# liuQuan98/EYOC

Hardware: AMD Instinct MI355X
Metric: registered pairs/sec (30k-voxel KITTI pairs) (higher is better)
Workload: dtype f32 (split16 products: fp32 storage/accumulation, 3 fp16 MFMAs on hi/lo-split operands per product); 1 GPU; 64 synthetic 30 cm KITTI-shaped pairs per step per GPU (mean 29894 voxels/cloud, ResUNetBN2C random-init, 5000-point NN, RANSAC 4000000 hypotheses/pair, planted inlier ratio 0.3, spconv math split16); parallelism=pairs sharded over 1 GPU(s), steps_in_flight=2

## Files before the change

### eyoc_amd/_lib.py

```python
from __future__ import annotations

import ctypes as C
import os
import threading

_HERE = os.path.dirname(os.path.abspath(__file__))
LIB_PATH = os.environ.get("EYOC_HIP_LIB") or os.path.join(_HERE, "lib", "libeyoc_hip.so")

MAX_LEVELS = 4
MAP_S1, MAP_DOWN, MAP_UP = 0, 1, 2


class MapsInfo(C.Structure):
    _fields_ = [("n_levels", C.c_int32), ("rows", C.c_int32 * MAX_LEVELS),
                ("pairs_s1", C.c_int64 * MAX_LEVELS), ("pairs_down", C.c_int64 * MAX_LEVELS),
                ("pairs_up", C.c_int64 * MAX_LEVELS), ("pairs_conv1", C.c_int64)]


class ModelDesc(C.Structure):
    _fields_ = [("in_channels", C.c_int32), ("out_channels", C.c_int32), ("conv1_kernel_size", C.c_int32),
                ("normalize_feature", C.c_int32), ("channels", C.c_int32 * 5), ("tr_channels", C.c_int32 * 5),
                ("bn_eps", C.c_float), ("expanded", C.c_int32)]


class LayerParams(C.Structure):
    _fields_ = [("name", C.c_char_p), ("kernel", C.POINTER(C.c_float)), ("K", C.c_int32), ("cin", C.c_int32),
                ("cout", C.c_int32), ("bias", C.POINTER(C.c_float)), ("bn_weight", C.POINTER(C.c_float)),
                ("bn_bias", C.POINTER(C.c_float)), ("bn_mean", C.POINTER(C.c_float)),
                ("bn_var", C.POINTER(C.c_float))]


class RansacParams(C.Structure):
    _fields_ = [("max_distance", C.c_float), ("edge_similarity", C.c_float), ("max_iteration", C.c_int32),
                ("seed", C.c_uint32)]


class RansacResult(C.Structure):
    _fields_ = [("T", C.c_float * 16), ("inliers", C.c_int32), ("best_hypothesis", C.c_int32),
                ("survivors", C.c_int32), ("inlier_rmse", C.c_float)]


class Sc2pcrParams(C.Structure):
    _fields_ = [("inlier_threshold", C.c_float), ("d_thre", C.c_float), ("ratio", C.c_float),
                ("nms_radius", C.c_float), ("num_iterations", C.c_int32), ("max_points", C.c_int32),
                ("k1", C.c_int32), ("k2", C.c_int32)]


_vp, _i, _sz = C.c_void_p, C.c_int, C.c_size_t
PROTOTYPES = {
    "eyoc_version": (_i, []),
    "eyoc_last_error": (C.c_char_p, []),
    "eyoc_create": (_i, [_i, C.POINTER(_vp)]),
    "eyoc_destroy": (_i, [_vp]),
    "eyoc_maps_workspace_bytes": (_sz, [_i]),
    "eyoc_maps_build": (_i, [_vp, _vp, _i, _vp, _sz, _vp, C.POINTER(_vp)]),
    "eyoc_maps_build_ordered": (_i, [_vp, _vp, _i, _vp, _sz, _vp, _i, C.POINTER(_vp)]),
    "eyoc_maps_free": (_i, [_vp]),
    "eyoc_maps_last_fault_batches": (_i, [_vp, _vp, _vp]),
    "eyoc_maps_internal_order": (_i, [_vp, _i]),
    "eyoc_maps_lazy_tables": (_i, [_vp, _i]),
    "eyoc_maps_fused_levels": (_i, [_vp, _i]),
    "eyoc_spconv_select_down_kernel": (_i, [_vp, _i]),
    "eyoc_maps_order_window_shift": (_i, [_vp, _i]),
    "eyoc_maps_row_order": (_vp, [_vp]),
    "eyoc_maps_copy_row_order": (_i, [_vp, _vp, _vp]),
    "eyoc_maps_rows": (_i, [_vp, _i]),
    "eyoc_maps_coords": (_vp, [_vp, _i]),
    "eyoc_maps_table": (_vp, [_vp, _i, _i]),
    "eyoc_maps_copy_coords": (_i, [_vp, _i, _vp, _vp]),
    "eyoc_maps_copy_table": (_i, [_vp, _i, _i, _vp, _vp]),
    "eyoc_maps_copy_up_order": (_i, [_vp, _i, _vp, _vp]),
    "eyoc_maps_order_min_rows": (_i, [_vp, _i]),
    "eyoc_maps_info": (_i, [_vp, _vp, _i, _vp, C.POINTER(MapsInfo)]),
    "eyoc_voxelize_workspace_bytes": (_sz, [_i]),
    "eyoc_voxelize": (_i, [_vp, _vp, _i, _i, C.c_float, _i, _vp, _vp, C.POINTER(C.c_int), _vp, _sz, _vp]),
    "eyoc_voxelize_batched_workspace_bytes": (_sz, [_i, _i]),
    "eyoc_voxelize_batched": (_i, [_vp, _vp, _i, C.POINTER(C.c_int64), _i, _i, C.c_float, _i, _vp, _vp, _vp,
                                   C.POINTER(C.c_int64), _vp, _sz, _vp]),
    "eyoc_voxelize_batched_isolating_workspace_bytes": (_sz, [_i, _i]),
    "eyoc_voxelize_batched_isolating": (_i, [_vp, _vp, _i, C.POINTER(C.c_int64), _i, _i, C.c_float, _i, _vp, _vp, _vp,
                                             C.POINTER(C.c_int64), _vp, _sz, _vp, _vp]),
    "eyoc_batch_drop_workspace_bytes": (_sz, [_i]),
    "eyoc_batch_drop": (_i, [_vp, _vp, _vp, _i, _i, _vp, _vp, _vp, _vp, C.POINTER(C.c_int), _vp, _vp, _sz, _vp]),
    "eyoc_remap_rows": (_i, [_vp, _vp, _i, _vp, _i, _vp, _vp]),
    "eyoc_gather_rows": (_i, [_vp, _vp, _i, _i, _vp, _i, _vp, C.c_float, _vp, _vp]),
    "eyoc_dotmax": (_i, [_vp, _vp, _vp, _i, C.POINTER(C.c_int32), C.POINTER(C.c_int32), _i, _vp, _vp, _vp]),
    "eyoc_knn2": (_i, [_vp, _vp, _vp, _i, C.POINTER(C.c_int32), C.POINTER(C.c_int32), _i, _vp, _vp, _vp, _vp]),
    "eyoc_lowe_topk": (_i, [_vp, _vp, _vp, _i, _i, _vp, _vp, _vp]),
    "eyoc_pair_filter": (_i, [_vp, _i, _vp, _vp, _vp, _vp, _i, _vp, C.c_float, _vp, _vp, _vp]),
    "eyoc_pair_filter_similarity": (_i, [_vp, _vp, _vp, _vp, _vp, _i, _vp, _i, _i, C.c_float, C.c_float, C.c_double, _vp, _vp,
                                         _vp]),
    "eyoc_spconv_packed_floats": (_sz, [_i, _i, _i]),
    "eyoc_spconv_pack_weights": (_i, [_vp, _vp, _i, _i, _i, _vp]),
    "eyoc_spconv_select_kernel": (_i, [_vp, _i]),
    "eyoc_spconv_pack_weights_transposed": (_i, [_vp, _i, _i, _i, _i, _vp]),
    "eyoc_spconv_grad_weight_workspace_bytes": (_sz, [_i, _i, _i, _i]),
    "eyoc_spconv_grad_weight": (_i, [_vp, _vp, _i, _i, _vp, _i, _i, _vp, _i, _i, _vp, _vp, _sz, _vp]),
    "eyoc_spconv_pack_weights_split16": (_i, [_vp, _vp, _i, _i, _i, _vp, _vp]),
    "eyoc_spconv_ex": (_i, [_vp, _vp, _i, _i, _i, _vp, _i, _i, _vp, _i, _vp, _vp, _i, _i, _vp, _i, _i, _i, _vp, _vp]),
    "eyoc_spconv_select_split16_kernel": (_i, [_vp, _i]),
    "eyoc_spconv_select_st_kernel": (_i, [_vp, _i]),
    "eyoc_spconv_st_split_below": (_i, [_vp, _i]),
    "eyoc_spconv_st_group_rows": (_i, [_vp, _i]),
    "eyoc_spconv_st_ksplit": (_i, [_vp, _i]),
    "eyoc_spconv_local_rulebook_bytes": (_sz, [_i]),
    "eyoc_spconv_build_local_rulebook": (_i, [_vp, _vp, _i, _i, _vp, _vp, _vp]),
    "eyoc_spconv_staged": (_i, [_vp, _vp, _vp, _i, _i, _vp, _i, _i, _vp, _i, _vp, _vp, _i, _i, _vp, _i, _i, _vp, _vp]),
    "eyoc_split16_encode": (_i, [_vp, _vp, _i, _i, _i, _vp, _i, _vp]),
    "eyoc_split16_decode": (_i, [_vp, _vp, _i, _i, _i, _vp, _i, _vp]),
    "eyoc_model_set_math": (_i, [_vp, _i]),
    "eyoc_model_last_math": (_i, [_vp]),
    "eyoc_model_range_check": (_i, [_vp, _vp, C.POINTER(C.c_float)]),
    "eyoc_model_range_snapshot": (_i, [_vp, _vp, _vp]),
    "eyoc_model_set_progress_event": (_i, [_vp, _i, _vp]),
    "eyoc_model_set_probe": (_i, [_vp, _i]),
    "eyoc_spconv": (_i, [_vp, _vp, _i, _i, _vp, _i, _i, _vp, _i, _vp, _vp, _i, _i, _vp, _i, _vp]),
    "eyoc_spconv_sum": (_i, [_vp, _vp, _i, _i, _vp, _i, _i, _vp, _i, _vp, _i, _vp]),
    "eyoc_model_blob_floats": (_sz, [C.POINTER(ModelDesc)]),
    "eyoc_model_pack_host": (_i, [C.POINTER(ModelDesc), C.POINTER(LayerParams), _i, _vp, _sz]),
    "eyoc_model_create": (_i, [_vp, C.POINTER(ModelDesc), C.POINTER(LayerParams), _i, _vp, _sz, C.POINTER(_vp)]),
    "eyoc_model_destroy": (_i, [_vp]),
    "eyoc_model_fuse_tail": (_i, [_vp, _i]),
    "eyoc_model_workspace_bytes": (_sz, [_vp, _vp]),
    "eyoc_model_forward": (_i, [_vp, _vp, _vp, _vp, _vp, _vp, _sz, _vp]),
    "eyoc_model_num_layers": (_i, [_vp]),
    "eyoc_model_layer_work": (_i, [_vp, _vp, _vp, _vp, C.POINTER(C.c_char_p), C.POINTER(C.c_int64),
                                   C.POINTER(C.c_double), C.POINTER(C.c_double), C.POINTER(C.c_double)]),
    "eyoc_model_set_timing": (_i, [_vp, _i]),
    "eyoc_model_layer_ms": (_i, [_vp, C.POINTER(C.c_float)]),
    "eyoc_model_timing_slot": (_i, [_vp, _i]),
    "eyoc_bn_workspace_bytes": (_sz, [_i, _i]),
    "eyoc_bn_train_forward": (_i, [_vp, _vp, _i, _i, _i, _vp, _vp, C.c_float, _i, _vp, _i, _vp, _vp, _sz, _vp]),
    "eyoc_bn_train_forward_running": (_i, [_vp, _vp, _i, _i, _i, _vp, _vp, C.c_float, _i, _vp, _i, _vp, _vp, _vp, C.c_float, _vp, _sz, _vp]),
    "eyoc_bn_train_backward": (_i, [_vp, _vp, _i, _vp, _i, _vp, _i, _i, _i, _vp, _vp, C.c_float, _vp, _i, _vp, _vp, _vp, _sz, _vp]),
    "eyoc_maps_gather_window": (_i, [_vp, _vp, _i, _vp, _i, _vp, _vp]),
    "eyoc_maps_gather_window_internal": (_i, [_vp, _vp, _i, _vp, _i, _vp, _vp]),
    "eyoc_knn_prefilter": (_i, [_vp, _i]),
    "eyoc_spconv_select_up_kernel": (_i, [_vp, _i]),
    "eyoc_spconv_upc_min_rows": (_i, [_vp, _i]),
    "eyoc_spconv_upc_tile_rows": (_i, [_i, _i]),
    "eyoc_spconv_upc_bytes": (_sz, [_i]),
    "eyoc_spconv_upc_build": (_i, [_vp, _vp, _i, _vp, _vp, _vp]),
    "eyoc_spconv_upc": (_i, [_vp, _vp, _vp, _i, _i, _vp, _i, _i, _vp, _i, _vp, _i, _vp, _i, _i, _vp, _vp]),
    "eyoc_spconv_select_conv1_kernel": (_i, [_vp, _i]),
    "eyoc_knn1": (_i, [_vp, _vp, _vp, _i, C.POINTER(C.c_int32), C.POINTER(C.c_int32), _i, _i, _vp, _vp, _vp]),
    "eyoc_pdist": (_i, [_vp, _vp, _i, _vp, _i, _i, _i, _vp, _vp]),
    "eyoc_kabsch_batched": (_i, [_vp, _vp, _vp, _vp, _i, _i, _vp, _vp]),
    "eyoc_irls_quad": (_i, [_vp, _vp, _vp, _vp, _i, _i, _vp, _vp]),
    "eyoc_ransac": (_i, [_vp, _vp, _vp, _vp, _i, C.POINTER(RansacParams), _vp, _vp]),
    "eyoc_maps_select_orders": (_i, [_vp, _i, _i]),
    "eyoc_ransac_select_pruning": (_i, [_vp, _i]),
    "eyoc_registration_accept_degenerate": (_i, [_vp, _i]),
    "eyoc_ransac_transform_store": (_i, [_vp, _i]),
    "eyoc_ransac_workspace_bytes": (_sz, [_vp, _i, _i, _i, _sz]),
    "eyoc_ransac_batched_ws": (_i, [_vp, _vp, _vp, _vp, C.POINTER(C.c_int32), C.POINTER(C.c_int32), _i,
                                    C.POINTER(RansacParams), _vp, _vp, _sz, _vp]),
    "eyoc_ransac_batched": (_i, [_vp, _vp, _vp, _vp, C.POINTER(C.c_int32), C.POINTER(C.c_int32), _i,
                                 C.POINTER(RansacParams), _vp, _vp]),
    "eyoc_sc2pcr_workspace_bytes": (_sz, [_i, C.POINTER(Sc2pcrParams)]),
    "eyoc_sc2pcr": (_i, [_vp, _vp, _vp, _i, C.POINTER(Sc2pcrParams), _vp, _vp, _vp, _sz, _vp]),
    "eyoc_sc2pcr_batched_workspace_bytes": (_sz, [_i, C.POINTER(Sc2pcrParams)]),
    "eyoc_sc2pcr_batched_workspace_bytes_n": (_sz, [_i, _i, C.POINTER(Sc2pcrParams)]),
    "eyoc_sc2pcr_set_shortlist_cap": (_i, [_vp, _i]),
    "eyoc_sc2pcr_set_dense_threshold": (_i, [_vp, _i]),
    "eyoc_sc2pcr_select_kernels": (_i, [_vp, _i]),
    "eyoc_sc2pcr_batched": (_i, [_vp, _vp, _vp, C.POINTER(C.c_int32), _i, C.POINTER(Sc2pcrParams), _vp, _vp, _i, _vp, _sz,
                                 _vp]),
}


ERR_INVALID, ERR_HIP, ERR_WORKSPACE, ERR_DUPLICATE, ERR_RANGE = -1, -2, -3, -4, -5


class EyocError(RuntimeError):

    def __init__(self, msg, code=None):
        super().__init__(msg)
        self.code = code


_lib = None
_lock = threading.Lock()
_ctx = {}


def load():
    global _lib
    if _lib is not None:
        return _lib
    with _lock:
        if _lib is None:
            if not os.path.exists(LIB_PATH):
                raise EyocError(
                    f"{LIB_PATH} not found: build it with `python -m eyoc_amd.build` (hipcc, gfx950). "
                    "There is no CPU fallback for this path.")
            lib = C.CDLL(LIB_PATH)
            for name, (res, args) in PROTOTYPES.items():
                fn = getattr(lib, name)
                fn.restype, fn.argtypes = res, args
            _lib = lib
    return _lib


def check(rc: int, what: str = ""):
    if rc != 0:
        msg = load().eyoc_last_error().decode("utf-8", "replace")
        raise EyocError(f"{what or 'libeyoc_hip'} failed ({rc}): {msg}", rc)


def ctx(device_index: int | None = None):
    import torch
    if device_index is not None:
        h = _ctx.get(device_index)
        if h is not None:
# ... 93 lines not shown
```

### eyoc_amd/csrc/common.h

```cpp
#pragma once
#include <hip/hip_runtime.h>

#include <cstdarg>
#include <cstdint>
#include <cstdio>
#include <cstring>
#include <string>
#include <vector>

#include "../../include/eyoc_hip.h"

namespace eyoc {

void set_error(const char* fmt, ...);

#define EYOC_CHECK_HIP(expr)                                                               \
  do {                                                                                     \
    hipError_t _e = (expr);                                                                \
    if (_e != hipSuccess) {                                                                \
      eyoc::set_error("%s failed: %s (%s:%d)", #expr, hipGetErrorString(_e), __FILE__,    \
                      __LINE__);                                                           \
      return EYOC_ERR_HIP;                                                                 \
    }                                                                                      \
  } while (0)

#define EYOC_REQUIRE(cond, code, ...)  \
  do {                                 \
    if (!(cond)) {                     \
      eyoc::set_error(__VA_ARGS__);    \
      return (code);                   \
    }                                  \
  } while (0)

inline size_t align_up(size_t v, size_t a = 256) { return (v + a - 1) / a * a; }
inline int cdiv(long long a, long long b) { return (int)((a + b - 1) / b); }

struct Carver {
  char* base;
  size_t off = 0, cap;
  Carver(void* p, size_t bytes) : base((char*)p), cap(bytes) {}
  template <typename T>
  T* take(size_t count) {
    size_t o = align_up(off);
    off = o + count * sizeof(T);
    return (T*)(base ? base + o : nullptr);
  }
  bool ok() const { return off <= cap; }
};

}

struct eyoc_ctx {
  int device = 0;
  void* scratch = nullptr;
  size_t scratch_bytes = 0;
  void* pinned = nullptr;
  size_t pinned_bytes = 0;
  int ensure_scratch(size_t bytes, hipStream_t st);
  hipStream_t scratch_owner = nullptr;
  bool scratch_owned = false;
  hipEvent_t scratch_ev = nullptr;
  static constexpr int POOL = 8;
  hipStream_t pool[POOL] = {};
  hipEvent_t pool_done[POOL] = {};
  hipEvent_t pool_fork = nullptr;
  bool pool_ready = false;
  int ensure_pool();
  bool ransac_attr_set = false, sc2_attr_set = false;
  bool up_attr_set[2] = {false, false};
  int zorder_kbits = 17, zorder_bbits = 10;
  int sc2_list_cap = 1024, sc2_dense_x = 0;
  int sc2_legacy = 0;
  uint32_t fault_dup[32] = {}, fault_range[32] = {};
  struct Knobs {
    int maps_order_min_rows = 65536;
    int maps_window_shift = 18;
    int maps_s1_order = 1, maps_down_order = 0;
    int maps_internal_order = -1;
    int maps_lazy_tables = 1, maps_fused_levels = 1;
    int knn_prefilter = 1;
    int fuse_tail = 2;
    int spconv_kernel = -1;
    int split16_kernel = 1;
    int up_kernel = 2;
    int s1_wide = 1;
    int st128_wide = 1;
    int down_kernel = 1;
    int upc_min_rows = 1 << 17;
    int conv1_kernel = 1;
    int st_group = 1;
    int st_variant = 1;
    int st_split_below = 1024;
    int st_cg_local = 1;
    int st_ksplit = 1;
    int ransac_store = 1 << 20;
    int ransac_prune = 2;
    int accept_degenerate = 0;
  } knobs;
};
inline const eyoc_ctx::Knobs& knobs_of(const eyoc_ctx* ctx) {
  static const eyoc_ctx::Knobs defaults;
  return ctx ? ctx->knobs : defaults;
}

namespace eyoc {

constexpr unsigned long long KEY_EMPTY = 0xFFFFFFFFFFFFFFFFull;
constexpr int COORD_BIAS = 1 << 17;
constexpr int VAL_UNSET = 0x7F7F7F7F;

struct HashTable {
  unsigned long long* keys;
  int* vals;
  unsigned int mask;
};

__host__ __device__ inline unsigned long long pack_key(int b, int x, int y, int z) {
  return ((unsigned long long)(unsigned)b << 54) |
         ((unsigned long long)((unsigned)(x + COORD_BIAS) & 0x3FFFFu) << 36) |
         ((unsigned long long)((unsigned)(y + COORD_BIAS) & 0x3FFFFu) << 18) |
         ((unsigned long long)((unsigned)(z + COORD_BIAS) & 0x3FFFFu));
}

__host__ __device__ inline unsigned int hash_key(unsigned long long k) {
  k ^= k >> 33;
  k *= 0xff51afd7ed558ccdull;
  k ^= k >> 33;
  k *= 0xc4ceb9fe1a85ec53ull;
  k ^= k >> 33;
  return (unsigned int)k;
}

__device__ inline int hash_lookup(const HashTable& t, unsigned long long key) {
  unsigned int s = hash_key(key) & t.mask;
  for (unsigned int probes = 0; probes <= t.mask; ++probes) {
    unsigned long long k = t.keys[s];
    if (k == key) return t.vals[s];
    if (k == KEY_EMPTY) return -1;
    s = (s + 1) & t.mask;
  }
  return -1;
}

}

struct eyoc_maps {
  int n_levels = 0;
  int rows[EYOC_MAX_LEVELS] = {0, 0, 0, 0};
  int32_t* coords[EYOC_MAX_LEVELS] = {nullptr, nullptr, nullptr, nullptr};
  eyoc::HashTable table[EYOC_MAX_LEVELS];
  int32_t* nbr_s1[EYOC_MAX_LEVELS] = {nullptr, nullptr, nullptr, nullptr};
  int32_t* nbr_down[EYOC_MAX_LEVELS] = {nullptr, nullptr, nullptr, nullptr};
  int32_t* nbr_up[EYOC_MAX_LEVELS] = {nullptr, nullptr, nullptr, nullptr};
  int32_t* parent[EYOC_MAX_LEVELS] = {nullptr, nullptr, nullptr, nullptr};
  int32_t* children[EYOC_MAX_LEVELS] = {nullptr, nullptr, nullptr, nullptr};
  int32_t* perm_up[EYOC_MAX_LEVELS] = {nullptr, nullptr, nullptr, nullptr};
  int32_t* perm_s1[EYOC_MAX_LEVELS] = {nullptr, nullptr, nullptr, nullptr};
  int32_t* perm_down[EYOC_MAX_LEVELS] = {nullptr, nullptr, nullptr, nullptr};
  int32_t* row_perm = nullptr;
  unsigned char* local_s1[EYOC_MAX_LEVELS] = {nullptr, nullptr, nullptr, nullptr};
  unsigned char* local_up[EYOC_MAX_LEVELS] = {nullptr, nullptr, nullptr, nullptr};
  unsigned char* local_s1w[EYOC_MAX_LEVELS] = {nullptr, nullptr, nullptr, nullptr};
  unsigned char* local_down[EYOC_MAX_LEVELS] = {nullptr, nullptr, nullptr, nullptr};
  unsigned char* local_upc[EYOC_MAX_LEVELS] = {nullptr, nullptr, nullptr, nullptr};
  bool table0_built = false;
  bool s1_ready[EYOC_MAX_LEVELS] = {true, true, true, true};
  bool up_ready[EYOC_MAX_LEVELS] = {true, true, true, true};
  int32_t* up8[EYOC_MAX_LEVELS] = {nullptr, nullptr, nullptr, nullptr};
  hipEvent_t s1_ev[EYOC_MAX_LEVELS] = {nullptr, nullptr, nullptr, nullptr};
  hipEvent_t up_ev[EYOC_MAX_LEVELS] = {nullptr, nullptr, nullptr, nullptr};
  hipEvent_t table0_ev = nullptr;
  eyoc_maps() = default;
  eyoc_maps(const eyoc_maps&) = delete;
  eyoc_maps& operator=(const eyoc_maps&) = delete;
  ~eyoc_maps();
};

namespace eyoc {
int maps_build_table0(eyoc_maps* maps, hipStream_t st);
int maps_ensure_table(eyoc_maps* maps, int kind, int level, hipStream_t st);
size_t sort_rows64_tmp_bytes(int n);
int sort_rows_by_key64(void* tmp, size_t tmp_bytes, const unsigned long long* keys_in, unsigned long long* keys_out, const int* vals_in,
                       int* vals_out, int n, int bits, hipStream_t st);
size_t sort_rows_tmp_bytes(int n, int bits);
int sort_rows_by_key(void* tmp, size_t tmp_bytes, const unsigned int* keys_in, unsigned int* keys_out, const int* vals_in,
                     int* vals_out, int n, int bits, hipStream_t st);
}
```

### eyoc_amd/csrc/coordmap.hip

```cpp
#include <cstdlib>

#include "spconv.h"
#include "derive.h"
#include "scan.h"

using namespace eyoc;

namespace {

__device__ inline void coarse_coord(const int32_t* c, int ts2, int& b, int& x, int& y, int& z) {
  const int m = ~(ts2 - 1);
  b = c[0]; x = c[1] & m; y = c[2] & m; z = c[3] & m;
}

__global__ void k_insert(const int32_t* __restrict__ coords, int n, int ts2, HashTable t, int* __restrict__ slot_out,
                         int* __restrict__ err, unsigned int* __restrict__ range_mask = nullptr) {
  int i = blockIdx.x * blockDim.x + threadIdx.x;
  if (i >= n) return;
  int b, x, y, z;
  coarse_coord(coords + 4 * (size_t)i, ts2, b, x, y, z);
  constexpr int LIM = COORD_BIAS - 16;
  if (b < 0 || b >= 1024 || x < -LIM || x >= LIM || y < -LIM || y >= LIM || z < -LIM || z >= LIM) {
    if (err) atomicAdd(&err[0], 1);
    if (range_mask && b >= 0 && b < 1024) atomicOr(&range_mask[b >> 5], 1u << (b & 31));
// ... 764 lines not shown
      hipLaunchKernelGGL(k_flag_sorted, dim3(cdiv(n_src, 256)), dim3(256), 0, st, src, n_src, ts2, flag,
                         l == 1 ? counters : (int*)nullptr, l == 1 ? counters + 1 : (int*)nullptr);
    } else {
      const unsigned int cap = table_capacity(n_src);
      t.keys = cv.take<unsigned long long>(cap);
      t.vals = cv.take<int>(cap);
      t.mask = cap - 1;
      FAIL_HIP(hipMemsetAsync(t.keys, 0xFF, (size_t)cap * 8, st));
      FAIL_HIP(hipMemsetAsync(t.vals, 0x7F, (size_t)cap * 4, st));
      hipLaunchKernelGGL(k_insert, dim3(cdiv(n_src, 256)), dim3(256), 0, st, src, n_src, ts2, t, slot, counters,
                         l == 1 ? fault_masks + 32 : (unsigned int*)nullptr);
      hipLaunchKernelGGL(k_flag, dim3(cdiv(n_src, 256)), dim3(256), 0, st, slot, t.vals, n_src, flag, (int*)nullptr);
    }
    hipLaunchKernelGGL(k_scan_partials, dim3(nb), dim3(SCAN_BLOCK), 0, st, flag, n_src, partial);
    hipLaunchKernelGGL(k_scan_top, dim3(1), dim3(SCAN_BLOCK), 0, st, partial, nb, counters + 2 + l);
    if (zorder) {
      m->rows[l] = pre_rows[l];
    } else {
    if (l == 1) {
      FAIL_HIP(hipMemcpyAsync(host + 128, counters, 128 * sizeof(int), hipMemcpyDeviceToHost, st));
      FAIL_HIP(hipStreamSynchronize(st));
      host[0] = host[128 + 2 + l]; host[1] = host[128]; host[2] = host[128 + 1];
    } else {
      FAIL_HIP(hipMemcpyAsync(host, counters + 2 + l, sizeof(int), hipMemcpyDeviceToHost, st));
      FAIL_HIP(hipStreamSynchronize(st));
    }
    if (l == 1 && host[1] != 0) {
      set_error("eyoc_maps_build: %d coordinate rows outside the supported key range (|c| < 2^17 - 16, 0 <= batch < 1024)", host[1]);
      keep_fault_masks(ctx, host + 128 + 64, EYOC_ERR_RANGE);
      delete m;
      return EYOC_ERR_RANGE;
    }
    if (l == 1 && sorted_level && host[2] != 0) {
      set_error("eyoc_maps_build: %d duplicate coordinate rows (a sparse tensor needs unique coordinates)", host[2]);
      keep_fault_masks(ctx, host + 128 + 64, EYOC_ERR_DUPLICATE);
      delete m;
      return EYOC_ERR_DUPLICATE;
    }
    m->rows[l] = host[0];
    }
    m->coords[l] = cv.take<int32_t>((size_t)m->rows[l] * 4);
    m->parent[l - 1] = cv.take<int32_t>((size_t)n_src);
    if (!zorder) {
      m->children[l - 1] = cv.take<int32_t>((size_t)m->rows[l] * 8);
      FAIL_HIP(hipMemsetAsync(m->children[l - 1], 0xFF, (size_t)m->rows[l] * 32, st));
    }
    if (sorted_level) {
      hipLaunchKernelGGL(k_compact_sorted, dim3(nb), dim3(SCAN_BLOCK), 0, st, flag, partial, src, n_src, ts2, l - 1,
                         m->coords[l], m->parent[l - 1], m->children[l - 1]);
      if (l + 1 == EYOC_MAX_LEVELS) {
        hipLaunchKernelGGL(k_insert, dim3(cdiv(m->rows[l], 256)), dim3(256), 0, st, m->coords[l], m->rows[l], ts2, t, (int*)nullptr, counters);
      }
      continue;
    }
    hipLaunchKernelGGL(k_compact<false>, dim3(nb), dim3(SCAN_BLOCK), 0, st, flag, partial, slot, src, n_src, ts2,
                       m->coords[l], t.vals, (int32_t*)nullptr);
    hipLaunchKernelGGL(k_children, dim3(cdiv(n_src, 256)), dim3(256), 0, st, slot, t.vals, src, n_src, l - 1,
                       m->parent[l - 1], m->children[l - 1], l == 1 ? counters + 1 : (int*)nullptr,
                       l == 1 ? fault_masks : (unsigned int*)nullptr);
    if (l == 1) {
      FAIL_HIP(hipMemcpyAsync(host + 128, counters, 128 * sizeof(int), hipMemcpyDeviceToHost, st));
      FAIL_HIP(hipStreamSynchronize(st));
      host[0] = host[128 + 1];
      if (host[0] != 0) {
        set_error("eyoc_maps_build: %d duplicate coordinate rows (a sparse tensor needs unique coordinates)", host[0]);
        keep_fault_masks(ctx, host + 128 + 64, EYOC_ERR_DUPLICATE);
        delete m;
        return EYOC_ERR_DUPLICATE;
      }
    }
  }
  const bool use_upc = kn.up_kernel == 2 && n >= kn.upc_min_rows;
  const bool use_up = kn.up_kernel == 1 || (kn.up_kernel == 2 && !use_upc);
  const bool lazy = zorder && use_upc && kn.maps_lazy_tables != 0;
  for (int l = 0; l < EYOC_MAX_LEVELS; ++l) {
    m->nbr_s1[l] = cv.take<int32_t>((size_t)27 * m->rows[l]);
    if (l + 1 < EYOC_MAX_LEVELS) {
      m->nbr_down[l] = cv.take<int32_t>((size_t)27 * m->rows[l + 1]);
      m->nbr_up[l] = cv.take<int32_t>((size_t)27 * m->rows[l]);
      if (lazy) {
        m->up8[l] = cv.take<int32_t>((size_t)8 * m->rows[l]);
        m->up_ready[l] = false;
      }
    }
  }
  if (lazy) m->s1_ready[0] = false;
  {
    const int top = EYOC_MAX_LEVELS - 1;
    hipLaunchKernelGGL(k_neighbours, dim3(cdiv(m->rows[top], 256)), dim3(256), 0, st, m->coords[top], m->rows[top],
                       m->table[top], 1 << top, 1, m->nbr_s1[top]);
  }
  const bool s1_order = kn.maps_s1_order != 0;
  int seg_up[EYOC_MAX_LEVELS], seg_s1[EYOC_MAX_LEVELS], seg_dn[EYOC_MAX_LEVELS], seg_base[3 * EYOC_MAX_LEVELS], n_seg = 0;
  size_t total = 0;
  for (int l = 0; l < EYOC_MAX_LEVELS; ++l) {
    seg_up[l] = seg_s1[l] = seg_dn[l] = -1;
    const bool dn_order = kn.maps_down_order == 1;
    if (l + 1 < EYOC_MAX_LEVELS && m->rows[l + 1] >= kn.maps_order_min_rows && (dn_order || !zorder)) {
      seg_dn[l] = n_seg; seg_base[n_seg++] = (int)total; total += m->rows[l + 1];
    }
    if (m->rows[l] < kn.maps_order_min_rows) continue;
    if (l + 1 < EYOC_MAX_LEVELS && !(zorder && (use_up || use_upc))) { seg_up[l] = n_seg; seg_base[n_seg++] = (int)total; total += m->rows[l]; }
    if (s1_order && !zorder) { seg_s1[l] = n_seg; seg_base[n_seg++] = (int)total; total += m->rows[l]; }
  }
  constexpr int TAG_SHIFT = UP_KEY_BITS, TAG_BITS = 4;
  const int wshift = zorder ? kn.maps_window_shift : -1;
  unsigned int* key_in = cv.take<unsigned int>(total);
  unsigned int* key_out = cv.take<unsigned int>(total);
  int* row_in = cv.take<int>(total);
  int32_t* perm_all = cv.take<int32_t>(total);
  const size_t sort_bytes = sort_rows_tmp_bytes((int)total, TAG_SHIFT + TAG_BITS);
  void* sort_tmp = cv.take<char>(sort_bytes);
  for (int l = EYOC_MAX_LEVELS - 2; l >= 0; --l) {
    const int nl = m->rows[l], nc = m->rows[l + 1];
    const int su = seg_up[l];
    if (lazy) {
      if (l > 0)
        hipLaunchKernelGGL((k_derive_fine<true, 2>), dim3(cdiv(nl, 256)), dim3(256), 0, st, m->coords[l], nl, l, m->parent[l], m->children[l],
                           m->nbr_s1[l + 1], nc, m->nbr_s1[l], m->up8[l], (unsigned int*)nullptr, (int*)nullptr, 0u, wshift);
    } else {
      hipLaunchKernelGGL((k_derive_fine<true, 1>), dim3(cdiv(nl, 256)), dim3(256), 0, st, m->coords[l], nl, l, m->parent[l],
                         m->children[l], m->nbr_s1[l + 1], nc, m->nbr_s1[l], m->nbr_up[l],
                         su >= 0 ? key_in + seg_base[su] : (unsigned int*)nullptr, su >= 0 ? row_in + seg_base[su] : (int*)nullptr,
                         (unsigned int)(su >= 0 ? su : 0) << TAG_SHIFT, wshift);
    }
    hipLaunchKernelGGL(k_derive_down, dim3(cdiv(nc, 256)), dim3(256), 0, st, nc, m->children[l], m->nbr_s1[l + 1],
                       m->nbr_down[l]);
  }
  for (int l = 0; l + 1 < EYOC_MAX_LEVELS; ++l) {
    const int sd = seg_dn[l];
    if (sd < 0) continue;
    hipLaunchKernelGGL(k_children_key, dim3(cdiv(m->rows[l + 1], 256)), dim3(256), 0, st, m->children[l], m->rows[l + 1],
                       key_in + seg_base[sd], row_in + seg_base[sd], (unsigned int)sd << TAG_SHIFT, wshift);
  }
  for (int l = 0; l < EYOC_MAX_LEVELS; ++l) {
    const int ss = seg_s1[l];
    if (ss < 0) continue;
    const int bits = l == 0 ? 2 : 4;
    hipLaunchKernelGGL(k_pattern_key, dim3(cdiv(m->rows[l], 256)), dim3(256), 0, st, m->nbr_s1[l], m->rows[l], bits,
                       key_in + seg_base[ss], row_in + seg_base[ss], (unsigned int)ss << TAG_SHIFT, wshift);
  }
  if (total > 0) {
    if (int rc = sort_rows_by_key(sort_tmp, sort_bytes, key_in, key_out, row_in, perm_all, (int)total, TAG_SHIFT + TAG_BITS, st)) {
      delete m;
      return rc;
    }
    for (int l = 0; l < EYOC_MAX_LEVELS; ++l) {
      if (seg_up[l] >= 0) m->perm_up[l] = perm_all + seg_base[seg_up[l]];
      if (seg_s1[l] >= 0) m->perm_s1[l] = perm_all + seg_base[seg_s1[l]];
      if (seg_dn[l] >= 0) m->perm_down[l] = perm_all + seg_base[seg_dn[l]];
    }
  }
  if (zorder) {
    for (int l = 0; l < EYOC_MAX_LEVELS; ++l) {
      m->local_s1[l] = cv.take<unsigned char>(local_rulebook_bytes(m->rows[l]));
      if (lazy && l == 0) {
        DeriveSrc src;
        src.coords = m->coords[0]; src.parent = m->parent[0]; src.children = m->children[0]; src.s1c = m->nbr_s1[1];
        src.nc = m->rows[1]; src.sh = 0; src.up8 = m->up8[0];
        if (int rc = build_local_rulebook_derived(src, m->rows[0], m->local_s1[0], counters + 8, st, kn.st_group)) { delete m; return rc; }
      } else if (int rc = build_local_rulebook(m->nbr_s1[l], 27, m->rows[l], m->local_s1[l], counters + 8, st, kn.st_group)) { delete m; return rc; }
      if (l + 1 < EYOC_MAX_LEVELS && use_up) {
        m->local_up[l] = cv.take<unsigned char>(local_rulebook_up_bytes(m->rows[l]));
        if (int rc = build_local_rulebook_up(m->nbr_up[l], 27, m->rows[l], m->local_up[l], counters + 9, st)) { delete m; return rc; }
      }
      if (l + 1 < EYOC_MAX_LEVELS && use_upc) {
        m->local_upc[l] = cv.take<unsigned char>(upc_kept_bytes(m->rows[l]));
        unsigned char* scratch = cv.take<unsigned char>(upc_scratch_bytes(m->rows[l]));
        if (m->local_upc[l]) {
          if (int rc = build_upc(lazy ? m->up8[l] : m->nbr_up[l], m->coords[l], 1 << l, m->rows[l], m->local_upc[l], scratch, st, lazy)) { delete m; return rc; }
        } else if (int rc = maps_ensure_table(m, EYOC_MAP_UP, l, st)) { delete m; return rc; }
      }
    }
    const bool use_down = kn.down_kernel == 1 && n >= kn.upc_min_rows;
    for (int l = EYOC_MAX_LEVELS - 1; l < EYOC_MAX_LEVELS && use_down && kn.s1_wide; ++l) {
      m->local_s1w[l] = cv.take<unsigned char>(local_rulebook128_bytes(m->rows[l]));
      if (m->local_s1w[l])
        if (int rc = build_local_rulebook128(m->nbr_s1[l], 27, m->rows[l], m->local_s1w[l], counters + 13, st, kn.st_group)) { delete m; return rc; }
    }
    for (int l = 0; l + 1 < EYOC_MAX_LEVELS && use_down; ++l) {
      m->local_down[l] = cv.take<unsigned char>(local_rulebook128_bytes(m->rows[l + 1]));
      if (m->local_down[l])
        if (int rc = build_local_rulebook128(m->nbr_down[l], 27, m->rows[l + 1], m->local_down[l], counters + 10 + l, st, kn.st_group)) { delete m; return rc; }
    }
    for (int l = 0; l < EYOC_MAX_LEVELS; ++l) {
      host[16 + l] = 0;
      if (m->local_upc[l]) FAIL_HIP(hipMemcpyAsync(host + 16 + l, upc_overflow_ptr(m->local_upc[l]), sizeof(int), hipMemcpyDeviceToHost, st));
    }
    FAIL_HIP(hipMemcpyAsync(host, counters + 8, 8 * sizeof(int), hipMemcpyDeviceToHost, st));
    FAIL_HIP(hipMemcpyAsync(host + 32, counters, 8 * sizeof(int), hipMemcpyDeviceToHost, st));
    FAIL_HIP(hipStreamSynchronize(st));
    if (host[32] != 0) {
      set_error("eyoc_maps_build: %d coordinate rows outside the supported key range (|c| < 2^17 - 16, 0 <= batch < 1024)", host[32]);
      keep_fault_masks(ctx, host + 64, EYOC_ERR_RANGE);
      delete m;
      return EYOC_ERR_RANGE;
    }
    if (host[33] != 0) {
      set_error("eyoc_maps_build: %d duplicate coordinate rows (a sparse tensor needs unique coordinates)", host[33]);
      keep_fault_masks(ctx, host + 64, EYOC_ERR_DUPLICATE);
      delete m;
      return EYOC_ERR_DUPLICATE;
    }
    for (int l = 1; l < EYOC_MAX_LEVELS; ++l)
      if (host[32 + 2 + l] != m->rows[l]) {
        set_error("eyoc_maps_build: internal error - level %d has %d rows by its scan, %d by the up-front count", l, host[32 + 2 + l], m->rows[l]);
        delete m;
        return EYOC_ERR_INVALID;
      }
    if (host[0] != 0) {
      for (int l = 0; l < EYOC_MAX_LEVELS; ++l) m->local_s1[l] = nullptr;
      if (int rc = maps_ensure_table(m, EYOC_MAP_S1, 0, st)) { delete m; return rc; }
    }
    if (host[1] != 0)
      for (int l = 0; l < EYOC_MAX_LEVELS; ++l) m->local_up[l] = nullptr;
    for (int l = 0; l + 1 < EYOC_MAX_LEVELS; ++l)
      if (host[2 + l] != 0) m->local_down[l] = nullptr;
    if (host[5] != 0)
      for (int l = 0; l < EYOC_MAX_LEVELS; ++l) m->local_s1w[l] = nullptr;
    for (int l = 0; l < EYOC_MAX_LEVELS; ++l)
      if (host[16 + l] != 0) {
        m->local_upc[l] = nullptr;
        if (int rc = maps_ensure_table(m, EYOC_MAP_UP, l, st)) { delete m; return rc; }
      }
  }
  FAIL_HIP(hipGetLastError());
#undef FAIL_HIP
  if (!cv.ok()) {
    set_error("eyoc_maps_build: internal workspace accounting error (%zu > %zu)", cv.off, cv.cap);
    delete m;
    return EYOC_ERR_WORKSPACE;
  }
  *out = m;
  return EYOC_OK;
}

size_t eyoc_voxelize_workspace_bytes(int n_points) {
  if (n_points < 0) return 0;
  const size_t n = (size_t)n_points, cap = table_capacity(n_points);
  return align_up(cap * 8) + align_up(cap * 4) + align_up(n * 16) + 3 * align_up(n * 4) +
         align_up((n / SCAN_TILE + 2) * 4) + 4096 + 16 * 256;
}

size_t eyoc_voxelize_batched_workspace_bytes(int n_points_total, int n_clouds) {
  if (n_points_total < 0 || n_clouds < 1) return 0;
  return eyoc_voxelize_workspace_bytes(n_points_total) + align_up((size_t)(n_clouds + 1) * 8) + align_up((size_t)(n_clouds + 1) * 4);
}

size_t eyoc_voxelize_batched_isolating_workspace_bytes(int n_points_total, int n_clouds) {
  if (n_points_total < 0 || n_clouds < 1) return 0;
  return eyoc_voxelize_batched_workspace_bytes(n_points_total, n_clouds) + align_up((size_t)n_clouds * 8 + 8);
}

}

namespace {

int voxelize_run(eyoc_ctx* ctx, const char* who, const float* xyz_dev, int n, int stride, const int64_t* pt_off_host,
                 int n_clouds, float voxel_size, int batch_base, int32_t* sel_dev, int32_t* coords_dev, float* xyz_out_dev,
                 int64_t* vox_off_host, void* ws, size_t ws_bytes, hipStream_t st, int32_t* faults_host = nullptr) {
  Carver cv(ws, ws_bytes);
  const bool iso = faults_host != nullptr;
  const int fo = 64 + ((n_clouds + 2) & ~1);
  int* counters = cv.take<int>(iso ? fo + 2 * n_clouds : 64 + n_clouds + 1);
  int* faults = counters + fo;
  int64_t* pt_off = cv.take<int64_t>(n_clouds + 1);
  int32_t* raw = cv.take<int32_t>((size_t)n * 4);
  int* slot = cv.take<int>(n);
  int* flag = cv.take<int>(n);
  int* partial = cv.take<int>(n / SCAN_TILE + 2);
  HashTable t;
  const unsigned int cap = table_capacity(n);
  t.keys = cv.take<unsigned long long>(cap);
  t.vals = cv.take<int>(cap);
  t.mask = cap - 1;
  EYOC_REQUIRE(cv.ok(), EYOC_ERR_WORKSPACE, "%s: internal workspace accounting error (%zu > %zu)", who, cv.off, cv.cap);
  const size_t up_bytes = n_clouds > 1 ? align_up((size_t)(n_clouds + 1) * 8) : 0;
  const int back = iso ? fo + 2 * n_clouds : n_clouds > 1 ? 64 + n_clouds + 1 : 4;
  EYOC_REQUIRE(up_bytes + (size_t)back * 4 <= ctx->pinned_bytes, EYOC_ERR_INVALID, "%s: %d clouds exceed the pinned staging", who,
               n_clouds);
  int64_t* up = (int64_t*)ctx->pinned;
  int* host = (int*)((char*)ctx->pinned + up_bytes);
  if (n_clouds > 1) {
    memcpy(up, pt_off_host, (size_t)(n_clouds + 1) * 8);
    EYOC_CHECK_HIP(hipMemcpyAsync(pt_off, up, (size_t)(n_clouds + 1) * 8, hipMemcpyHostToDevice, st));
  }
  EYOC_CHECK_HIP(hipMemsetAsync(counters, 0, 64 * sizeof(int), st));
  if (iso) EYOC_CHECK_HIP(hipMemsetAsync(faults, 0, (size_t)n_clouds * 2 * sizeof(int), st));
  EYOC_CHECK_HIP(hipMemsetAsync(t.keys, 0xFF, (size_t)cap * 8, st));
  EYOC_CHECK_HIP(hipMemsetAsync(t.vals, 0x7F, (size_t)cap * 4, st));
  if (iso) {
    hipLaunchKernelGGL(k_quantize<true>, dim3(cdiv(n, 256)), dim3(256), 0, st, xyz_dev, n, stride, voxel_size, (const int64_t*)pt_off,
                       n_clouds, batch_base, raw, counters + 1, faults);
    hipLaunchKernelGGL(k_insert_runs<true>, dim3(cdiv(n, 256)), dim3(256), 0, st, (const int32_t*)raw, n, t, slot, counters,
                       (const int*)faults, batch_base);
  } else {
    hipLaunchKernelGGL(k_quantize<false>, dim3(cdiv(n, 256)), dim3(256), 0, st, xyz_dev, n, stride, voxel_size, (const int64_t*)pt_off,
                       n_clouds, batch_base, raw, counters + 1, (int*)nullptr);
    hipLaunchKernelGGL(k_insert_runs<false>, dim3(cdiv(n, 256)), dim3(256), 0, st, (const int32_t*)raw, n, t, slot, counters,
                       (const int*)nullptr, 0);
  }
  hipLaunchKernelGGL(k_flag, dim3(cdiv(n, 256)), dim3(256), 0, st, slot, t.vals, n, flag, (int*)nullptr);
  const int nb = cdiv(n, SCAN_TILE);
  hipLaunchKernelGGL(k_scan_partials, dim3(nb), dim3(SCAN_BLOCK), 0, st, flag, n, partial);
  hipLaunchKernelGGL(k_scan_top, dim3(1), dim3(SCAN_BLOCK), 0, st, partial, nb, counters + 2);
  if (n_clouds > 1)
    hipLaunchKernelGGL(k_cloud_offsets, dim3(cdiv(n_clouds + 1, 4)), dim3(256), 0, st, (const int*)flag, (const int*)partial,
                       (const int*)(counters + 2), n, (const int64_t*)pt_off, n_clouds, counters + 64);
  hipLaunchKernelGGL(k_compact<true>, dim3(nb), dim3(SCAN_BLOCK), 0, st, flag, partial, slot, raw, n, 1, coords_dev, t.vals,
                     sel_dev, (const int64_t*)pt_off, n_clouds, batch_base, xyz_dev, stride, xyz_out_dev);
  EYOC_CHECK_HIP(hipGetLastError());
  EYOC_CHECK_HIP(hipMemcpyAsync(host, counters, (size_t)back * sizeof(int), hipMemcpyDeviceToHost, st));
  EYOC_CHECK_HIP(hipStreamSynchronize(st));
  if (host[0] != 0) {
    if (n_clouds > 1)
      EYOC_REQUIRE(false, EYOC_ERR_RANGE, "%s: %d points fall outside the key range (|c| < 2^17 - 16), the first of them in cloud %d",
                   who, host[0], n_clouds - host[1]);
    EYOC_REQUIRE(false, EYOC_ERR_RANGE, "%s: %d points fall outside the key range (|c| < 2^17 - 16)", who, host[0]);
  }
  if (iso) memcpy(faults_host, host + fo, (size_t)n_clouds * 2 * sizeof(int));
  vox_off_host[0] = 0;
  if (n_clouds == 1) {
    vox_off_host[1] = host[2];
  } else {
    for (int b = 1; b <= n_clouds; ++b) vox_off_host[b] = host[64 + b];
  }
  return EYOC_OK;
}

}

extern "C" {

// ... 48 lines not shown
                      sel_dev, coords_dev, xyz_out_dev, voxel_offsets, ws, ws_bytes, (hipStream_t)stream, cloud_faults);
}

int eyoc_voxelize_batched(eyoc_ctx* ctx, const float* xyz_dev, int stride, const int64_t* point_offsets, int n_clouds,
                          int n_points, float voxel_size, int batch_base, int32_t* sel_dev, int32_t* coords_dev,
                          float* xyz_out_dev, int64_t* voxel_offsets, void* ws, size_t ws_bytes, void* stream) {
  return voxelize_batched("eyoc_voxelize_batched", false, ctx, xyz_dev, stride, point_offsets, n_clouds, n_points, voxel_size,
                          batch_base, sel_dev, coords_dev, xyz_out_dev, voxel_offsets, ws, ws_bytes, stream, nullptr);
}

int eyoc_voxelize_batched_isolating(eyoc_ctx* ctx, const float* xyz_dev, int stride, const int64_t* point_offsets, int n_clouds,
                                    int n_points, float voxel_size, int batch_base, int32_t* sel_dev, int32_t* coords_dev,
                                    float* xyz_out_dev, int64_t* voxel_offsets, void* ws, size_t ws_bytes, void* stream,
                                    int32_t* cloud_faults) {
  return voxelize_batched("eyoc_voxelize_batched_isolating", true, ctx, xyz_dev, stride, point_offsets, n_clouds, n_points,
                          voxel_size, batch_base, sel_dev, coords_dev, xyz_out_dev, voxel_offsets, ws, ws_bytes, stream, cloud_faults);
}

int eyoc_maps_free(eyoc_maps* maps) {
  delete maps;
  return EYOC_OK;
}

int eyoc_maps_rows(const eyoc_maps* maps, int level) {
  if (!maps || level < 0 || level >= maps->n_levels) return -1;
  return maps->rows[level];
}

const int32_t* eyoc_maps_coords(const eyoc_maps* maps, int level) {
  if (!maps || level < 0 || level >= maps->n_levels) return nullptr;
  return maps->coords[level];
}

const int32_t* eyoc_maps_table(const eyoc_maps* maps, int kind, int level) {
  const int32_t* t = table_ptr(maps, kind, level);
  if (!t) return nullptr;
  eyoc_maps* mm = const_cast<eyoc_maps*>(maps);
  if (hipEvent_t* ev = fill_event(mm, kind, level)) {
    if ((kind == EYOC_MAP_S1 ? !maps->s1_ready[level] : !maps->up_ready[level]) && maps_ensure_table(mm, kind, level, (hipStream_t)nullptr) != EYOC_OK)
      return nullptr;
    if (*ev && hipEventSynchronize(*ev) != hipSuccess) return nullptr;
  }
  return t;
}

int eyoc_maps_copy_coords(const eyoc_maps* maps, int level, int32_t* out_dev, void* stream) {
  const int32_t* src = eyoc_maps_coords(maps, level);
  EYOC_REQUIRE(src && out_dev, EYOC_ERR_INVALID, "eyoc_maps_copy_coords: bad level %d or NULL output", level);
  EYOC_CHECK_HIP(hipMemcpyAsync(out_dev, src, (size_t)maps->rows[level] * 16, hipMemcpyDeviceToDevice, (hipStream_t)stream));
  return EYOC_OK;
}

int eyoc_maps_copy_table(const eyoc_maps* maps, int kind, int level, int32_t* out_dev, void* stream) {
  const int32_t* src = table_ptr(maps, kind, level);
  EYOC_REQUIRE(src && out_dev, EYOC_ERR_INVALID, "eyoc_maps_copy_table: bad kind %d / level %d or NULL output", kind, level);
  if (int rc = maps_ensure_table(const_cast<eyoc_maps*>(maps), kind, level, (hipStream_t)stream)) return rc;
  const int n_out = kind == EYOC_MAP_DOWN ? maps->rows[level + 1] : maps->rows[level];
  EYOC_CHECK_HIP(hipMemcpyAsync(out_dev, src, (size_t)n_out * 27 * 4, hipMemcpyDeviceToDevice, (hipStream_t)stream));
  return EYOC_OK;
}

}

static int publish_fill(hipEvent_t& ev, hipStream_t st) {
  if (!ev) EYOC_CHECK_HIP(hipEventCreateWithFlags(&ev, hipEventDisableTiming));
  EYOC_CHECK_HIP(hipEventRecord(ev, st));
  return EYOC_OK;
}

int eyoc::maps_ensure_table(eyoc_maps* m, int kind, int level, hipStream_t st) {
  hipEvent_t* ev = fill_event(m, kind, level);
  if (!ev) return EYOC_OK;
  bool& ready = (kind == EYOC_MAP_S1 ? m->s1_ready : m->up_ready)[level];
  if (ready) {
    if (*ev) EYOC_CHECK_HIP(hipStreamWaitEvent(st, *ev, 0));
    return EYOC_OK;
  }
  const int nl = m->rows[level], nc = m->rows[level + 1];
  if (nl > 0) {
    if (kind == EYOC_MAP_S1)
      hipLaunchKernelGGL((k_derive_fine<true, 0>), dim3(cdiv(nl, 256)), dim3(256), 0, st, m->coords[level], nl, level, m->parent[level],
                         m->children[level], m->nbr_s1[level + 1], nc, m->nbr_s1[level], (int32_t*)nullptr, (unsigned int*)nullptr,
                         (int*)nullptr, 0u, -1);
    else
      hipLaunchKernelGGL((k_derive_fine<false, 1>), dim3(cdiv(nl, 256)), dim3(256), 0, st, m->coords[level], nl, level, m->parent[level],
                         m->children[level], m->nbr_s1[level + 1], nc, (int32_t*)nullptr, m->nbr_up[level], (unsigned int*)nullptr,
                         (int*)nullptr, 0u, -1);
    EYOC_CHECK_HIP(hipGetLastError());
  }
  if (int rc = publish_fill(*ev, st)) return rc;
  ready = true;
  return EYOC_OK;
}

int eyoc::maps_build_table0(eyoc_maps* m, hipStream_t st) {
  if (m->table0_built) {
    if (m->table0_ev) EYOC_CHECK_HIP(hipStreamWaitEvent(st, m->table0_ev, 0));
    return EYOC_OK;
  }
  HashTable& t = m->table[0];
  const size_t cap = (size_t)t.mask + 1;
  EYOC_CHECK_HIP(hipMemsetAsync(t.keys, 0xFF, cap * 8, st));
  EYOC_CHECK_HIP(hipMemsetAsync(t.vals, 0x7F, cap * 4, st));
  hipLaunchKernelGGL(k_insert, dim3(cdiv(m->rows[0], 256)), dim3(256), 0, st, m->coords[0], m->rows[0], 1, t, (int*)nullptr,
                     (int*)nullptr );
  EYOC_CHECK_HIP(hipGetLastError());
  if (int rc = publish_fill(m->table0_ev, st)) return rc;
  m->table0_built = true;
  return EYOC_OK;
}

eyoc_maps::~eyoc_maps() {
  for (hipEvent_t* ev : {&table0_ev, s1_ev + 0, s1_ev + 1, s1_ev + 2, s1_ev + 3, up_ev + 0, up_ev + 1, up_ev + 2, up_ev + 3})
    if (*ev) {
      (void)hipEventSynchronize(*ev);
      (void)hipEventDestroy(*ev);
    }
}

extern "C" {

int eyoc_maps_last_fault_batches(const eyoc_ctx* ctx, uint32_t* dup, uint32_t* range) {
  EYOC_REQUIRE(ctx && dup && range, EYOC_ERR_INVALID, "eyoc_maps_last_fault_batches: NULL argument");
  memcpy(dup, ctx->fault_dup, sizeof(ctx->fault_dup));
  memcpy(range, ctx->fault_range, sizeof(ctx->fault_range));
  return EYOC_OK;
}

int eyoc_maps_internal_order(eyoc_ctx* ctx, int mode) {
  if (!ctx) return -1;
  const int prev = ctx->knobs.maps_internal_order;
  if (mode >= -1 && mode <= 1) ctx->knobs.maps_internal_order = mode;
  return prev + 2;
}

const int32_t* eyoc_maps_row_order(const eyoc_maps* maps) { return maps ? maps->row_perm : nullptr; }

int eyoc_spconv_select_down_kernel(eyoc_ctx* ctx, int mode) {
  EYOC_REQUIRE(ctx, EYOC_ERR_INVALID, "eyoc_spconv_select_down_kernel: NULL ctx");
  const int prev = ctx->knobs.down_kernel;
  if (mode == 0 || mode == 1) ctx->knobs.down_kernel = mode;
  if (mode == 2 || mode == 3) ctx->knobs.st128_wide = mode - 2;
  if (mode == 4 || mode == 5) ctx->knobs.s1_wide = mode - 4;
  return prev;
}

int eyoc_maps_lazy_tables(eyoc_ctx* ctx, int on) {
  EYOC_REQUIRE(ctx, EYOC_ERR_INVALID, "eyoc_maps_lazy_tables: NULL ctx");
  const int prev = ctx->knobs.maps_lazy_tables;
  if (on == 0 || on == 1) ctx->knobs.maps_lazy_tables = on;
  return prev;
}

int eyoc_maps_fused_levels(eyoc_ctx* ctx, int on) {
  EYOC_REQUIRE(ctx, EYOC_ERR_INVALID, "eyoc_maps_fused_levels: NULL ctx");
  const int prev = ctx->knobs.maps_fused_levels;
  if (on == 0 || on == 1) ctx->knobs.maps_fused_levels = on;
  return prev;
}

int eyoc_maps_select_orders(eyoc_ctx* ctx, int s1, int down) {
  if (!ctx) return -1;
  eyoc_ctx::Knobs& kn = ctx->knobs;
  const int prev = kn.maps_s1_order | kn.maps_down_order << 1;
  if (s1 == 0 || s1 == 1) kn.maps_s1_order = s1;
  if (down == 0 || down == 1) kn.maps_down_order = down;
  return prev;
}

int eyoc_maps_order_window_shift(eyoc_ctx* ctx, int shift) {
  if (!ctx) return -1;
  const int prev = ctx->knobs.maps_window_shift;
  if (shift >= 0) ctx->knobs.maps_window_shift = shift;
  return prev;
}

int eyoc_maps_order_min_rows(eyoc_ctx* ctx, int min_rows) {
  if (!ctx) return -1;
  const int prev = ctx->knobs.maps_order_min_rows;
  if (min_rows >= 0) ctx->knobs.maps_order_min_rows = min_rows;
  return prev;
}

int eyoc_maps_copy_up_order(const eyoc_maps* maps, int level, int32_t* out_dev, void* stream) {
  EYOC_REQUIRE(maps && out_dev && level >= 0 && level + 1 < maps->n_levels, EYOC_ERR_INVALID,
               "eyoc_maps_copy_up_order: bad level %d or NULL argument", level);
  const int n = maps->rows[level];
  if (maps->perm_up[level]) {
    EYOC_CHECK_HIP(hipMemcpyAsync(out_dev, maps->perm_up[level], (size_t)n * 4, hipMemcpyDeviceToDevice, (hipStream_t)stream));
  } else {
    hipLaunchKernelGGL(k_iota, dim3(cdiv(n, 256)), dim3(256), 0, (hipStream_t)stream, out_dev, n);
    EYOC_CHECK_HIP(hipGetLastError());
  }
  return EYOC_OK;
}

int eyoc_maps_copy_row_order(const eyoc_maps* maps, int32_t* out_dev, void* stream) {
  EYOC_REQUIRE(maps && out_dev, EYOC_ERR_INVALID, "eyoc_maps_copy_row_order: NULL argument");
  const int n = maps->rows[0];
  if (maps->row_perm) {
    EYOC_CHECK_HIP(hipMemcpyAsync(out_dev, maps->row_perm, (size_t)n * 4, hipMemcpyDeviceToDevice, (hipStream_t)stream));
  } else {
    hipLaunchKernelGGL(k_iota, dim3(cdiv(n, 256)), dim3(256), 0, (hipStream_t)stream, out_dev, n);
    EYOC_CHECK_HIP(hipGetLastError());
  }
  return EYOC_OK;
}

int eyoc_maps_info(eyoc_ctx* ctx, const eyoc_maps* m, int conv1_ks, void* stream, eyoc_maps_info_t* info) {
  EYOC_REQUIRE(ctx && m && info, EYOC_ERR_INVALID, "eyoc_maps_info: NULL argument");
  hipStream_t st = (hipStream_t)stream;
  int rc = ctx->ensure_scratch(64 * sizeof(unsigned long long), st);
  if (rc) return rc;
  unsigned long long* cnt = (unsigned long long*)ctx->scratch;
  EYOC_CHECK_HIP(hipMemsetAsync(cnt, 0, 64 * sizeof(unsigned long long), st));
  memset(info, 0, sizeof(*info));
  info->n_levels = m->n_levels;
  auto count = [&](const int32_t* t, long long n, int slot) {
    if (!t || n == 0) return;
    int blocks = (int)((n + 1023) / 1024);
    if (blocks > 2048) blocks = 2048;
    hipLaunchKernelGGL(k_count_valid, dim3(blocks), dim3(256), 0, st, t, n, cnt + slot);
  };
  for (int l = 0; l < m->n_levels; ++l) {
    info->rows[l] = m->rows[l];
    if ((rc = maps_ensure_table(const_cast<eyoc_maps*>(m), EYOC_MAP_S1, l, st))) return rc;
    if (l + 1 < m->n_levels && (rc = maps_ensure_table(const_cast<eyoc_maps*>(m), EYOC_MAP_UP, l, st))) return rc;
    count(m->nbr_s1[l], 27ll * m->rows[l], l);
    if (l + 1 < m->n_levels) {
      count(m->nbr_down[l], 27ll * m->rows[l + 1], 8 + l);
      count(m->nbr_up[l], 27ll * m->rows[l], 16 + l);
    }
  }
  if (conv1_ks > 0) {
    rc = maps_build_table0(const_cast<eyoc_maps*>(m), st);
    if (rc) return rc;
    hipLaunchKernelGGL(k_count_region, dim3(cdiv(m->rows[0], 256)), dim3(256), 0, st, m->coords[0], m->rows[0],
                       m->table[0], conv1_ks, cnt + 24);
  }
  unsigned long long* host = (unsigned long long*)ctx->pinned;
  EYOC_CHECK_HIP(hipMemcpyAsync(host, cnt, 32 * sizeof(unsigned long long), hipMemcpyDeviceToHost, st));
  EYOC_CHECK_HIP(hipStreamSynchronize(st));
  for (int l = 0; l < m->n_levels; ++l) {
    info->pairs_s1[l] = (int64_t)host[l];
    info->pairs_down[l] = (int64_t)host[8 + l];
    info->pairs_up[l] = (int64_t)host[16 + l];
  }
  info->pairs_conv1 = (int64_t)host[24];
  return EYOC_OK;
}

}
```

### eyoc_amd/csrc/spconv.h

```cpp
#pragma once
#include "common.h"

namespace eyoc {

inline int spconv_ct(int cout) { return cout >= 128 ? 128 : cout; }
inline int spconv_cc(int cin, int ) { return cin % 64 == 0 ? 64 : 32; }

struct TailFuse {
  const float* skip = nullptr;
  int ld_skip = 0;
  const float *w1 = nullptr, *s1 = nullptr, *b1 = nullptr, *w2 = nullptr, *s2 = nullptr, *b2 = nullptr;
  int relu1 = 0, l2norm = 0;
  float* out = nullptr;
  int ld_out = 0;
  const int32_t* out_perm = nullptr;
};

struct SpconvArgs {
  const int32_t* nbr;
  int K, n_out;
  int n_in = 0;
  const float* in;
  int ld_in, cin;
  const float* w;
  int cout;
  const float* bias;
  const float* res;
  int ld_res;
  int relu;
  int l2norm;
  float* out;
  int ld_out;
  int math = 0;
  int out_split = 0;
  const int32_t* out_perm = nullptr;
  const unsigned char* local = nullptr;
  const unsigned char* local128 = nullptr;
  const unsigned char* local_down = nullptr;
  const unsigned char* local_up = nullptr;
  const unsigned char* local_upc = nullptr;
  const float* out_scale = nullptr;
  const int32_t* perm = nullptr;
  int small_rows = 0;
  unsigned int* range = nullptr;
  eyoc_ctx* ctx = nullptr;
  float* ks_part = nullptr;
  int allow_offset_split = 0, offset_split = 1;
  float* offset_part = nullptr;
  int cg_local = 0;
  TailFuse tail;
};
constexpr int KS_MAX_SLOTS = 1024;
constexpr size_t KS_PART_BYTES = (size_t)KS_MAX_SLOTS * 256 * 32 * 4;

typedef _Float16 half8_t __attribute__((ext_vector_type(8)));
typedef _Float16 half4_t __attribute__((ext_vector_type(4)));

__device__ inline void split16_encode4(const float4 v, uint2& hi, uint2& lo) {
  half4_t h, l;
  h[0] = (_Float16)v.x; h[1] = (_Float16)v.y; h[2] = (_Float16)v.z; h[3] = (_Float16)v.w;
  l[0] = (_Float16)(v.x - (float)h[0]); l[1] = (_Float16)(v.y - (float)h[1]);
  l[2] = (_Float16)(v.z - (float)h[2]); l[3] = (_Float16)(v.w - (float)h[3]);
  hi = __builtin_bit_cast(uint2, h);
  lo = __builtin_bit_cast(uint2, l);
}
__device__ inline float4 split16_decode4(const uint2 hi, const uint2 lo) {
  const half4_t h = __builtin_bit_cast(half4_t, hi), l = __builtin_bit_cast(half4_t, lo);
  return make_float4((float)h[0] + (float)l[0], (float)h[1] + (float)l[1], (float)h[2] + (float)l[2], (float)h[3] + (float)l[3]);
}
__host__ __device__ inline int split16_off4(int c) { return (c >> 5) * 128 + (c & 31) * 2; }
constexpr int SPLIT16_LO = 64;
__device__ inline void split16_store4(float* row, int c, const float4 v) {
  uint2 hi, lo;
  split16_encode4(v, hi, lo);
  char* p = reinterpret_cast<char*>(row) + split16_off4(c);
  *reinterpret_cast<uint2*>(p) = hi;
  *reinterpret_cast<uint2*>(p + SPLIT16_LO) = lo;
}
__device__ inline float4 split16_load4(const float* row, int c) {
  const char* p = reinterpret_cast<const char*>(row) + split16_off4(c);
  return split16_decode4(*reinterpret_cast<const uint2*>(p), *reinterpret_cast<const uint2*>(p + SPLIT16_LO));
}

constexpr float SPLIT16_LIMIT = 6.0e4f;
__device__ inline float split16_merge(float a, float b) {
  const unsigned int x = __float_as_uint(a) & 0x7FFFFFFFu, y = __float_as_uint(b) & 0x7FFFFFFFu;
  return __uint_as_float(x > y ? x : y);
}
__device__ inline bool split16_over(float mx) { return (__float_as_uint(mx) & 0x7FFFFFFFu) >= __float_as_uint(SPLIT16_LIMIT); }
__device__ inline void split16_track(float& mx, const float4 v) {
  mx = split16_merge(split16_merge(split16_merge(mx, v.x), split16_merge(v.y, v.z)), v.w);
}
__device__ inline void split16_report(unsigned int* range, float mx) {
  if (!range) return;
  if (split16_over(mx)) { atomicOr(range, 1u); atomicOr(range + 3, 1u); }
  if (__builtin_nontemporal_load(range + 2)) atomicMax(range + 1, __float_as_uint(mx) & 0x7FFFFFFFu);
}
__device__ inline bool split16_poisoned(const unsigned int* range) { return range && __builtin_nontemporal_load(range) != 0u; }

__device__ __forceinline__ void lds_barrier() { asm volatile("s_waitcnt lgkmcnt(0)\n\ts_barrier" ::: "memory"); }

template <int HS>
__device__ inline int canonical_slot_id(const int* hk, const unsigned short* hpos, int s) {
  const int kv = hk[s];
  int start = s, len = 1;
  while (len < HS && hk[(start - 1) & (HS - 1)] >= 0) { start = (start - 1) & (HS - 1); ++len; }
  int rank = 0;
  for (int q = start; q != s; q = (q + 1) & (HS - 1)) rank += hk[q] < kv;
  for (int q = (s + 1) & (HS - 1); hk[q] >= 0 && q != start; q = (q + 1) & (HS - 1)) rank += hk[q] < kv;
  return hpos[(start + rank) & (HS - 1)];
}

int launch_spconv(const SpconvArgs& a, hipStream_t st);
int launch_permute_rows(const float* in, const int32_t* perm, int n, int c, float* out, hipStream_t st);
int launch_spconv_st(const SpconvArgs& a, const unsigned char* local_dev, hipStream_t st);
int launch_spconv_up(const SpconvArgs& a, const unsigned char* local_dev, hipStream_t st);
size_t local_rulebook_up_bytes(int n_out);
bool spconv_st_can_fuse_tail(const SpconvArgs& a);
int spconv_record_path(const SpconvArgs& a);
int build_local_rulebook_up(const int32_t* nbr_dev, int K, int n_out, unsigned char* out_dev, int* overflow_dev, hipStream_t st);
size_t upc_kept_bytes(int n_out);
size_t upc_scratch_bytes(int n_out);
int build_upc(const int32_t* nbr_dev, const int32_t* coords_dev, int stride, int n_out, unsigned char* ws, unsigned char* scratch, hipStream_t st, bool compact = false);
const int* upc_overflow_ptr(const unsigned char* ws);
int upc_set_tile_rows(int odd_axes, int rows);
int launch_spconv_upc(const SpconvArgs& a, const unsigned char* ws, hipStream_t st);
int st_variants();
size_t local_rulebook_bytes(int n_out);
int build_local_rulebook(const int32_t* nbr_dev, int K, int n_out, unsigned char* out_dev, int* overflow_dev, hipStream_t st, int group = 1);
struct DeriveSrc {
  const int32_t* coords = nullptr;
  const int32_t* parent = nullptr;
  const int32_t* children = nullptr;
  const int32_t* s1c = nullptr;
  int nc = 0, sh = 0;
  int32_t* up8 = nullptr;
};
size_t local_rulebook128_bytes(int n_out);
int build_local_rulebook128(const int32_t* nbr_dev, int K, int n_out, unsigned char* out_dev, int* overflow_dev, hipStream_t st, int group = 1);
int launch_spconv_st128(const SpconvArgs& a, const unsigned char* local_dev, hipStream_t st);
int build_local_rulebook_derived(const DeriveSrc& src, int n_out, unsigned char* out_dev, int* overflow_dev, hipStream_t st, int group = 1);
int launch_spconv_rs(const SpconvArgs& a, hipStream_t st);
bool tail_fusable(int cin1, int cmid, int cout);
int launch_tail_fused(const float* in, int ld_in, int n, const float* w1, const float* s1, const float* b1, int relu1, const float* w2,
                      const float* s2, const float* b2, int l2norm, float* out, int ld_out, const int32_t* out_perm, unsigned int* range,
                      hipStream_t st);
bool spconv_rs_fits(const SpconvArgs& a);
int launch_spconv_wave(const SpconvArgs& a, hipStream_t st);

struct Conv1Args {
  const int32_t* coords;
  int n;
  HashTable table;
  int ks;
  const float* in;
  int cin;
  const float* w;
  const float* bias;
  int cout;
  const float* wscale = nullptr;
  float* out;
  int ld_out;
  int out_split = 0;
  unsigned int* range = nullptr;
  const int32_t* in_perm = nullptr;
  const int32_t* parent;
  const int32_t* children;
  const int32_t* s1c;
  int nc;
  const unsigned char* local1 = nullptr;
  const eyoc_ctx* ctx = nullptr;
};
constexpr int ST_TILE = 256, ST_UMAX = 639, ST_UCAP = 1280, ST_NPASS = 2, ST_LOC_OFF = 16 + ST_UCAP * 4, ST_INV_OFF = 33152, ST_LR_BYTES = 33408;
int launch_conv1(const Conv1Args& a, hipStream_t st);
bool conv1_walks_octree(const Conv1Args& a);

}
```

### eyoc_amd/csrc/spconv_st.hip

```cpp
#include <atomic>
#include <cstdlib>

#include "spconv.h"
#include "derive.h"

using namespace eyoc;

namespace {

typedef float f32x4 __attribute__((ext_vector_type(4)));
typedef unsigned int u32x4 __attribute__((ext_vector_type(4)));

constexpr int NW = 4;
constexpr int TILE = NW * 64;
constexpr int XROWS = 640;
constexpr int UMAX = XROWS - 1;
constexpr int NPASS = 2;
constexpr int UCAP = 1280;
constexpr int X_BYTES = XROWS * 128;
constexpr int LO_REGION = XROWS * 64;
constexpr int NIT = XROWS / (16 * NW);
__host__ __device__ constexpr int slot_addr(int l) { return l * 64 + ((l >> 2) & 3) * 16; }

constexpr int MASK_OFF = 16 + UCAP * 4 + NPASS * 27 * 64 * 8;
constexpr int MASK_PASS_BYTES = 56;
constexpr int RM_OFF = MASK_OFF + NPASS * MASK_PASS_BYTES;
constexpr int INV_OFF = RM_OFF + TILE;
constexpr int LR_BYTES = INV_OFF + TILE;
static_assert(INV_OFF == ST_INV_OFF, "spconv.h mirrors this layout");
static_assert(TILE == ST_TILE && UMAX == ST_UMAX && UCAP == ST_UCAP && NPASS == ST_NPASS && LR_BYTES == ST_LR_BYTES, "spconv.h mirrors this layout");
static_assert(LR_BYTES % 128 == 0, "records start on cache lines");
#ifndef EYOC_LR_HSLOTS_LOG2
#define EYOC_LR_HSLOTS_LOG2 11
#endif
constexpr int HSLOTS_LOG2 = EYOC_LR_HSLOTS_LOG2, HSLOTS_T = 1 << HSLOTS_LOG2;

template <bool DERIVE, int NWB>
__global__ __launch_bounds__(NWB * 64) void k_local_rulebook(const int32_t* __restrict__ nbr, int K, int n_out, unsigned char* __restrict__ out,
                                                             int* __restrict__ overflow, int group, DeriveSrc d) {
  constexpr int TR = NWB * 64;
  constexpr int HS = HSLOTS_T, HSHIFT = 32 - HSLOTS_LOG2;
  __shared__ int hk[HS];
  __shared__ unsigned short hid[HS];
  __shared__ unsigned short srow[27][TR];
  __shared__ __attribute__((aligned(16))) unsigned long long key[TR];
  __shared__ int wave_cnt[NWB];
  __shared__ int too_many;
  const int lane = threadIdx.x & 63, wave = threadIdx.x >> 6;
  const int tile = blockIdx.x;
  const int row = tile * TR + (int)threadIdx.x;
  for (int i = threadIdx.x; i < HS; i += TR) hk[i] = -1;
  if (threadIdx.x == 0) too_many = 0;
  __syncthreads();
  unsigned short slot[27];
  int idxs[27];
  if constexpr (DERIVE) {
#pragma unroll
    for (int k = 0; k < 27; ++k) idxs[k] = -1;
    if (row < n_out) {
      const int4 c = reinterpret_cast<const int4*>(d.coords)[row];
      const int b[3] = {(c.y >> d.sh) & 1, (c.z >> d.sh) & 1, (c.w >> d.sh) & 1};
      int blk[8];
      derive_blocks(b, d.parent[row], d.s1c, d.nc, blk);
      derive_window(b, blk, d.children, idxs);
      if (d.up8) {
        int bl[8];
        derive_up_blocks(b, blk, bl);
        const int cls = b[0] | (b[1] << 1) | (b[2] << 2);
#pragma unroll
        for (int m = 0; m < 8; ++m) d.up8[(size_t)m * n_out + row] = (m & ~cls) == 0 ? bl[m] : -1;
      }
    }
  } else {
#pragma unroll
    for (int k = 0; k < 27; ++k) idxs[k] = (k < K && row < n_out) ? nbr[(size_t)k * n_out + row] : -1;
  }
#pragma unroll
  for (int k = 0; k < 27; ++k) {
    const int idx = idxs[k];
    unsigned int s = 0xFFFFu;
    if (idx >= 0) {
      s = ((unsigned)idx * 2654435761u) >> HSHIFT;
      int probes = 0;
      while (true) {
        const int prev = atomicCAS(&hk[s], -1, idx);
        if (prev == -1 || prev == idx) break;
        s = (s + 1) & (HS - 1);
        if (++probes >= HS) { too_many = 1; s = 0xFFFFu; break; }
      }
    }
    slot[k] = (unsigned short)s;
  }
  {
    unsigned int mask = 0;
#pragma unroll
    for (int k = 0; k < 27; ++k) {
      srow[k][threadIdx.x] = slot[k];
      if (slot[k] != 0xFFFFu) mask |= 1u << k;
    }
    const unsigned int zp = (mask >> 18) & 0x1FFu, zm = mask & 0x1FFu, z0 = (mask >> 9) & 0x1FFu;
    const unsigned int yp = mask & 0x70381C0u ? 1u : 0u;
    const unsigned int ym = mask & 0x01C0E07u ? 1u : 0u;
    const unsigned int xp = mask & 0x4924924u ? 1u : 0u;
    const unsigned int xm = mask & 0x1249249u ? 1u : 0u;
    unsigned int cb = (zp ? 32u : 0u) | (zm ? 16u : 0u) | (yp << 3) | (ym << 2) | (xp << 1) | xm;
    cb ^= cb >> 1; cb ^= cb >> 2; cb ^= cb >> 4;
    const unsigned long long coarse = cb;
    const unsigned long long pattern = ((unsigned long long)zp << 18) | ((unsigned long long)zm << 9) | z0;
    key[threadIdx.x] = group ? (coarse << 35) | (pattern << 8) | threadIdx.x : (unsigned long long)threadIdx.x;
  }
  __syncthreads();
  if (too_many) {
    if (threadIdx.x == 0) {
      reinterpret_cast<int*>(out + (size_t)tile * LR_BYTES)[0] = -1;
      atomicAdd(overflow, 1);
    }
    return;
  }
  constexpr int PER_WAVE = HS / NWB;
  int cnt = 0;
  for (int i0 = 0; i0 < PER_WAVE; i0 += 64) cnt += __popcll(__ballot(hk[wave * PER_WAVE + i0 + lane] >= 0));
  if (lane == 0) wave_cnt[wave] = cnt;
  __syncthreads();
  int base = 0, total = 0;
  for (int w = 0; w < NWB; ++w) { if (w < wave) base += wave_cnt[w]; total += wave_cnt[w]; }
  unsigned char* lr = out + (size_t)tile * LR_BYTES;
  int* U = reinterpret_cast<int*>(lr + 16);
  if (total <= UMAX) {
    for (int i0 = 0; i0 < PER_WAVE; i0 += 64) {
      const int s = wave * PER_WAVE + i0 + lane;
      const int key = hk[s];
      const unsigned long long m = __ballot(key >= 0);
      const int id = base + __popcll(m & ((1ull << lane) - 1ull));
      if (key >= 0) {
        hid[s] = (unsigned short)id;
        U[id] = key;
      }
      base += __popcll(m);
    }
  } else {
    for (int i0 = 0; i0 < PER_WAVE; i0 += 64) {
      const int s = wave * PER_WAVE + i0 + lane;
      const unsigned long long m = __ballot(hk[s] >= 0);
      if (hk[s] >= 0) hid[s] = (unsigned short)(base + __popcll(m & ((1ull << lane) - 1ull)));
      base += __popcll(m);
    }
    __syncthreads();
    unsigned short ids[PER_WAVE / 64];
#pragma unroll
    for (int q = 0; q < PER_WAVE / 64; ++q) {
      const int s = wave * PER_WAVE + q * 64 + lane;
      ids[q] = hk[s] >= 0 ? (unsigned short)canonical_slot_id<HS>(hk, hid, s) : (unsigned short)0;
    }
    __syncthreads();
#pragma unroll
    for (int q = 0; q < PER_WAVE / 64; ++q) {
      const int s = wave * PER_WAVE + q * 64 + lane;
      const int key = hk[s];
      if (key >= 0) {
        hid[s] = ids[q];
        if (ids[q] < NPASS * UMAX) U[ids[q]] = key;
      }
    }
  }
  if (threadIdx.x == 0) {
    reinterpret_cast<int*>(lr)[0] = total <= NPASS * UMAX ? total : -1;
    if (total > NPASS * UMAX) atomicAdd(overflow, 1);
  }
  __syncthreads();
  if (group) {
    const unsigned long long mine = key[threadIdx.x];
    int rank = 0;
    const ulonglong2* kp = reinterpret_cast<const ulonglong2*>(key);
#pragma unroll 8
    for (int i = 0; i < TR / 2; ++i) {
      const ulonglong2 kk = kp[i];
      rank += (kk.x < mine) + (kk.y < mine);
    }
    __syncthreads();
    key[rank] = mine;
    __syncthreads();
  }
  unsigned short* loc = reinterpret_cast<unsigned short*>(lr + 16 + UCAP * 4);
  unsigned char* msk = lr + MASK_OFF;
  __shared__ unsigned char nib[NPASS][27][4];
  const int r = (int)threadIdx.x, w = r >> 6, c = (r >> 4) & 3, j = r & 15;
  const int src = (int)(key[group ? (c * NWB + ((c & 1) ? NWB - 1 - w : w)) * 16 + j : r] & 255u);
  lr[RM_OFF + (w * 16 + j) * 4 + c] = (unsigned char)src;
  lr[INV_OFF + src] = (unsigned char)r;
#pragma unroll
  for (int k = 0; k < 27; ++k) {
    const unsigned int hs = srow[k][src];
    const int id = hs != 0xFFFFu ? (int)hid[hs] : -1;
#pragma unroll
    for (int p = 0; p < NPASS; ++p) {
      if (p > 0 && total <= p * UMAX) continue;
      const int l = (id >= p * UMAX && id < (p + 1) * UMAX) ? id - p * UMAX : UMAX;
      loc[(((size_t)(p * 27 + k) * 64) + w * 16 + j) * 4 + c] = (unsigned short)slot_addr(l);
      const unsigned long long b = __ballot(l != UMAX);
      if (lane == 0)
        nib[p][k][w] = (unsigned char)(((b & 0xFFFFull) != 0) | (((b >> 16) & 0xFFFFull) != 0) << 1 | (((b >> 32) & 0xFFFFull) != 0) << 2 |
                                       (((b >> 48) & 0xFFFFull) != 0) << 3);
    }
  }
  __syncthreads();
  if (threadIdx.x < NPASS * 28) {
    const int p = (int)threadIdx.x / 28, k = (int)threadIdx.x % 28;
    unsigned short m = 0;
    if (k < 27 && !(p > 0 && total <= p * UMAX)) {
      m = (unsigned short)(nib[p][k][0] | nib[p][k][1] << 4);
      if (NWB == 4) m |= (unsigned short)(nib[p][k][2] << 8 | nib[p][k][3] << 12);
    }
    reinterpret_cast<unsigned short*>(msk)[p * 28 + k] = m;
  }
}

template <int NTW, int CC, int NH>
__global__ __launch_bounds__(NW * 64, 2) void spconv_st_kernel(SpconvArgs a, const unsigned char* __restrict__ local, int n_tiles) {
  constexpr int CTW = NTW * 16, NC = 4;
  constexpr int CTG = CTW * NH;
  constexpr int WD = (NTW * NH <= 2) ? 2 : 1;
  extern __shared__ __attribute__((aligned(16))) unsigned char xs[];
  const int lane = threadIdx.x & 63;
  const int wave = __builtin_amdgcn_readfirstlane((int)(threadIdx.x >> 6));
  const int g = lane >> 4, j = lane & 15;
  const int n_cg = a.cout / CTG;
  const int xcd = (int)blockIdx.x & 7, per = 8 / n_cg;
  const int cg = xcd % n_cg, tile = ((int)blockIdx.x >> 3) * per + xcd / n_cg;
  if (tile >= n_tiles) return;
  const int w0 = NH == 1 ? wave : 2 * (wave >> 1);
  const int ct0 = cg * CTG + (NH == 2 ? (wave & 1) * CTW : 0);
  const int CT = a.cout >= 128 ? 128 : a.cout;
  const int n_slices = a.cout / CT, slice = ct0 / CT, nt0 = (ct0 - slice * CT) / 16;
  constexpr int JQ = CC / 16;
  const int ncc = a.cin / CC;
  const int nqb = a.cin / 32;
  constexpr int K = 27;

  const unsigned char* lr = local + (size_t)tile * LR_BYTES;
  const int n_u = __builtin_amdgcn_readfirstlane(reinterpret_cast<const int*>(lr)[0]);
  const int* __restrict__ U = reinterpret_cast<const int*>(lr + 16);
  const uint2* __restrict__ locp = reinterpret_cast<const uint2*>(lr + 16 + UCAP * 4) + w0 * 16 + j;
  const int n_pass = n_u > UMAX ? 2 : 1;
  if (threadIdx.x < 8)
    *reinterpret_cast<float4*>(xs + (threadIdx.x >> 2) * LO_REGION + UMAX * 64 + (threadIdx.x & 3) * 16) = make_float4(0.f, 0.f, 0.f, 0.f);

  const __amdgpu_buffer_rsrc_t wrsrc = __builtin_amdgcn_make_buffer_rsrc(const_cast<float*>(a.w), 0, K * a.cin * a.cout * 4, 0x00020000);
  const int tile4 = CC * CT / 4;

  f32x4 acc[NH][NC][NTW];
#pragma unroll
  for (int h = 0; h < NH; ++h)
#pragma unroll
    for (int c = 0; c < NC; ++c)
#pragma unroll
      for (int t = 0; t < NTW; ++t) acc[h][c][t] = f32x4{0.f, 0.f, 0.f, 0.f};

  const int lane_off = lane * 16;
  auto load_w = [&](int k, int qb, float4 (&W)[NTW][2]) {
    const int cc = (qb * 32) / CC, qp = ((qb * 32) % CC) / 32;
    const int wbase = __builtin_amdgcn_readfirstlane((((k * n_slices + slice) * ncc + cc) * tile4 + (nt0 * JQ + 2 * qp) * 64) * 16);
#if defined(EYOC_ST_ABL) && (EYOC_ST_ABL & 4)
    for (int t = 0; t < NTW; ++t) { asm volatile("" : "+v"(W[t][0].x), "+v"(W[t][1].x)); }
    return;
#endif
#pragma unroll
    for (int t = 0; t < NTW; ++t)
#pragma unroll
      for (int p = 0; p < 2; ++p) {
        const u32x4 v = __builtin_amdgcn_raw_buffer_load_b128(wrsrc, lane_off + (t * JQ + p) * 1024, wbase, 0);
        W[t][p] = make_float4(__uint_as_float(v.x), __uint_as_float(v.y), __uint_as_float(v.z), __uint_as_float(v.w));
      }
  };
  int n_up = 0;
  auto stage = [&](int pass, int qb) {
#if defined(EYOC_ST_ABL) && (EYOC_ST_ABL & 2)
    return;
#endif
    int Ureg[NIT];
#pragma unroll
    for (int it = 0; it < NIT; ++it) {
      int l = (it * NW + wave) * 16 + (lane >> 2);
      asm volatile("" : "+v"(l));
      Ureg[it] = l < n_up ? U[pass * UMAX + l] : 0;
    }
#pragma unroll
    for (int it = 0; it < NIT; ++it) {
      const int l0 = (it * NW + wave) * 16;
      if (l0 < n_up) {
        const int l = l0 + (lane >> 2);
        const float* src = a.in + (size_t)Ureg[it] * a.ld_in + qb * 32 + (((lane & 3) ^ ((l >> 2) & 3)) << 2);
        if (l < n_up) {
          __builtin_amdgcn_global_load_lds(src, (__attribute__((address_space(3))) void*)(xs + l0 * 64), 16, 0, 0);
          __builtin_amdgcn_global_load_lds(src + 16, (__attribute__((address_space(3))) void*)(xs + LO_REGION + l0 * 64), 16, 0, 0);
        }
      }
    }
  };
  const unsigned int gh = (unsigned)g << 4;
  auto read_x = [&](const uint2 L, float4 (&X)[NC][2]) {
#if defined(EYOC_ST_ABL) && (EYOC_ST_ABL & 8)
    for (int c = 0; c < NC; ++c) { X[c][0].x = __uint_as_float(L.x); asm volatile("" : "+v"(X[c][0].y), "+v"(X[c][1].x)); }
    return;
#endif
#pragma unroll
    for (int c = 0; c < NC; ++c) {
      const unsigned int ad = (((c < 2 ? L.x : L.y) >> (16 * (c & 1))) & 0xFFFFu) ^ gh;
      X[c][0] = *reinterpret_cast<const float4*>(xs + ad);
      X[c][1] = *reinterpret_cast<const float4*>(xs + ad + LO_REGION);
    }
  };
  auto multiply = [&](int h, const float4 (&X)[NC][2], const float4 (&W)[NTW][2]) {
#pragma unroll
    for (int term = 0; term < 3; ++term)
#pragma unroll
      for (int c = 0; c < NC; ++c) {
        const half8_t xv = __builtin_bit_cast(half8_t, X[c][term == 1 ? 1 : 0]);
#pragma unroll
        for (int t = 0; t < NTW; ++t)
          acc[h][c][t] = __builtin_amdgcn_mfma_f32_16x16x32_f16(__builtin_bit_cast(half8_t, W[t][term == 2 ? 1 : 0]), xv, acc[h][c][t], 0, 0, 0);
      }
  };

  float4 XA[NC][2], XB[NC][2], W[3][NTW][2];
  uint2 L[3][NH];
  bool first = true;
  for (int pass = 0; pass < n_pass; ++pass) {
    n_up = min(n_u - pass * UMAX, UMAX);
    const uint2* lp = locp + pass * 27 * 64;
    for (int qb = 0; qb < nqb; ++qb) {
      if (!first) __syncthreads();
      first = false;
      stage(pass, qb);
      load_w(0, qb, W[0]);
      if (WD == 2) load_w(1, qb, W[1]);
#pragma unroll
      for (int h = 0; h < NH; ++h) { L[0][h] = lp[h * 16]; L[1][h] = lp[64 + h * 16]; }
      __builtin_amdgcn_s_waitcnt(0x0070);
      __syncthreads();
      read_x(L[0][0], XA);
#pragma unroll
      for (int hs = 0; hs < 27 * NH; ++hs) {
        const int k = hs / NH, h = hs % NH;
        if (h == 0 && k + 2 < 27) {
#pragma unroll
          for (int hh = 0; hh < NH; ++hh) L[(k + 2) % 3][hh] = lp[(k + 2) * 64 + hh * 16];
        }
        if (h == 0 && k + WD < 27) load_w(k + WD, qb, W[(k + WD) % 3]);
        const int hn = hs + 1, kn = hn / NH, hhn = hn % NH;
        if (hs & 1) {
          if (hn < 27 * NH) read_x(L[kn % 3][hhn], XA);
          multiply(h, XB, W[k % 3]);
        } else {
          if (hn < 27 * NH) read_x(L[kn % 3][hhn], XB);
          multiply(h, XA, W[k % 3]);
        }
#if defined(EYOC_ST_ABL) && (EYOC_ST_ABL & 256)
        __builtin_amdgcn_sched_group_barrier(0x020, 8, 0);
#pragma unroll
        for (int i = 0; i < 4; ++i) {
          __builtin_amdgcn_sched_group_barrier(0x008, 6, 0);
          __builtin_amdgcn_sched_group_barrier(0x100, 2, 0);
        }
#endif
#if !(defined(EYOC_ST_ABL) && (EYOC_ST_ABL & 128))
        __builtin_amdgcn_sched_barrier(0);
#endif
// ... 357 lines not shown
    float4 b1[4], b2[2];
#pragma unroll
    for (int t = 0; t < 4; ++t) b1[t] = *reinterpret_cast<const float4*>(tf.b1 + 16 * t + 4 * g);
#pragma unroll
    for (int t = 0; t < 2; ++t) b2[t] = *reinterpret_cast<const float4*>(tf.b2 + 16 * t + 4 * g);
    lds_barrier();
    unsigned char* xw = xs + (size_t)(wave * NK) * 2048 + lane * 16;
#pragma unroll
    for (int k = 0; k < NK; ++k) {
      *reinterpret_cast<uint4*>(xw + k * 2048) = sel4(odd, Xh[k], Xh[NK + k]);
      *reinterpret_cast<uint4*>(xw + k * 2048 + 1024) = sel4(odd, Xl[k], Xl[NK + k]);
    }
    lds_barrier();
    const unsigned char* xr = xs + (size_t)((wave ^ 1) * NK) * 2048 + lane * 16;
    uint4 Ph[NK], Pl[NK];
#pragma unroll
    for (int k = 0; k < NK; ++k) {
      Ph[k] = *reinterpret_cast<const uint4*>(xr + k * 2048);
      Pl[k] = *reinterpret_cast<const uint4*>(xr + k * 2048 + 1024);
    }
    f32x4 acc1[NK][4];
#pragma unroll
    for (int k = 0; k < NK; ++k)
#pragma unroll
      for (int t = 0; t < 4; ++t) acc1[k][t] = f32x4{0.f, 0.f, 0.f, 0.f};
#pragma unroll
    for (int cc = 0; cc < 3; ++cc) {
      if (cc < 2) load_w1(cc + 1, Wc[(cc + 1) & 1]);
      else load_w2();
#pragma unroll
      for (int k = 0; k < NK; ++k) {
        const bool mine = cc == (odd ? 1 : 0);
        const uint4 xh = cc == 2 ? Sh[k] : sel4(mine, Oh[k], Ph[k]), xl = cc == 2 ? Sl[k] : sel4(mine, Ol[k], Pl[k]);
        const half8_t X0 = __builtin_bit_cast(half8_t, xh), X1 = __builtin_bit_cast(half8_t, xl);
#pragma unroll
        for (int term = 0; term < 3; ++term)
#pragma unroll
          for (int t = 0; t < 4; ++t)
            acc1[k][t] = __builtin_amdgcn_mfma_f32_16x16x32_f16(Wc[cc & 1][t][term == 2 ? 1 : 0], term == 1 ? X1 : X0, acc1[k][t], 0, 0, 0);
      }
    }
    const bool poisoned = split16_poisoned(a.range) || split16_over(mx);
    const float qnan = __builtin_nanf("");
    float mx2 = 0.f;
#pragma unroll
    for (int k = 0; k < NK; ++k) {
      half8_t Y[2][2];
      float cmx = 0.f;
#pragma unroll
      for (int t = 0; t < 4; ++t) {
        float4 u = make_float4(acc1[k][t][0] * os1 + b1[t].x, acc1[k][t][1] * os1 + b1[t].y, acc1[k][t][2] * os1 + b1[t].z, acc1[k][t][3] * os1 + b1[t].w);
        if (tf.relu1) { u.x = fmaxf(u.x, 0.f); u.y = fmaxf(u.y, 0.f); u.z = fmaxf(u.z, 0.f); u.w = fmaxf(u.w, 0.f); }
        split16_track(cmx, u);
        uint2 h, l;
        split16_encode4(u, h, l);
        const half4_t h4 = __builtin_bit_cast(half4_t, h), l4 = __builtin_bit_cast(half4_t, l);
#pragma unroll
        for (int r = 0; r < 4; ++r) { Y[t >> 1][0][4 * (t & 1) + r] = h4[r]; Y[t >> 1][1][4 * (t & 1) + r] = l4[r]; }
      }
      f32x4 o2[2];
#pragma unroll
      for (int t = 0; t < 2; ++t) o2[t] = f32x4{0.f, 0.f, 0.f, 0.f};
#pragma unroll
      for (int kb = 0; kb < 2; ++kb)
#pragma unroll
        for (int term = 0; term < 3; ++term)
#pragma unroll
          for (int t = 0; t < 2; ++t)
            o2[t] = __builtin_amdgcn_mfma_f32_16x16x32_f16(W2[t][kb][term == 2 ? 1 : 0], Y[kb][term == 1 ? 1 : 0], o2[t], 0, 0, 0);
      float4 w[2];
      float ss = 0.f;
#pragma unroll
      for (int t = 0; t < 2; ++t) {
        w[t] = make_float4(o2[t][0] * os2 + b2[t].x, o2[t][1] * os2 + b2[t].y, o2[t][2] * os2 + b2[t].z, o2[t][3] * os2 + b2[t].w);
        ss += w[t].x * w[t].x + w[t].y * w[t].y + w[t].z * w[t].z + w[t].w * w[t].w;
      }
      if (tf.l2norm) {
        ss += __shfl_xor(ss, 16, 64);
        ss += __shfl_xor(ss, 32, 64);
        const float inv = 1.0f / sqrtf(ss);
#pragma unroll
        for (int t = 0; t < 2; ++t) { w[t].x *= inv; w[t].y *= inv; w[t].z *= inv; w[t].w *= inv; }
      }
      if (myrow[k] < a.n_out) mx2 = split16_merge(mx2, cmx);
      cmx = split16_merge(cmx, __shfl_xor(cmx, 16, 64));
      cmx = split16_merge(cmx, __shfl_xor(cmx, 32, 64));
      const bool bad = poisoned || split16_over(cmx);
      if (myrow[k] < a.n_out) {
        const size_t oo = tf.out_perm ? (size_t)tf.out_perm[myrow[k]] : (size_t)myrow[k];
#pragma unroll
        for (int t = 0; t < 2; ++t)
          *reinterpret_cast<float4*>(tf.out + oo * tf.ld_out + 16 * t + 4 * g) = bad ? make_float4(qnan, qnan, qnan, qnan) : w[t];
      }
    }
    if (a.range) {
      if (split16_over(mx)) { atomicOr(a.range + 4, 1u); atomicOr(a.range + 3, 1u); }
      if (split16_over(mx2)) { atomicOr(a.range + 5, 1u); atomicOr(a.range + 3, 1u); }
      if (__builtin_nontemporal_load(a.range + 2)) atomicMax(a.range + 1, __float_as_uint(split16_merge(mx, mx2)) & 0x7FFFFFFFu);
    }
    return;
  }
#pragma unroll
  for (int hc = 0; hc < NG; ++hc) {
    const int o = orow[hc];
    if (o >= a.n_out) continue;
    if (SKIP == 7 && os != 12345.f) continue;
    if (a.out_split) {
      uint2 h0, l0, h1, l1;
      split16_encode4(v[hc][0], h0, l0);
      split16_encode4(v[hc][1], h1, l1);
      char* op = reinterpret_cast<char*>(a.out + (size_t)o * a.ld_out) + split16_off4(ch);
      *reinterpret_cast<uint4*>(op) = make_uint4(h0.x, h0.y, h1.x, h1.y);
      *reinterpret_cast<uint4*>(op + SPLIT16_LO) = make_uint4(l0.x, l0.y, l1.x, l1.y);
    } else {
      float* op = a.out + (size_t)o * a.ld_out + ch;
      *reinterpret_cast<float4*>(op) = v[hc][0];
      *reinterpret_cast<float4*>(op + 4) = v[hc][1];
    }
  }
  if (a.out_split) split16_report(a.range, mx);
#ifdef EYOC_ST_TRACE
  asm volatile("s_waitcnt vmcnt(0)" ::: "memory");
  ST_STAMP(8);
  if (threadIdx.x == 0 && blockIdx.x < TRACE_WGS) {
    unsigned int hw;
    asm volatile("s_getreg_b32 %0, hwreg(HW_REG_HW_ID)" : "=s"(hw));
    unsigned int xcc;
    asm volatile("s_getreg_b32 %0, hwreg(HW_REG_XCC_ID)" : "=s"(xcc));
    g_st_trace[blockIdx.x * TRACE_N + 9] = ((unsigned long long)xcc << 32) | hw;
  }
#endif
}

}

#ifdef EYOC_ST_TRACE
extern "C" int eyoc_debug_st_trace(unsigned long long* host, size_t n) {
  if (n > (size_t)TRACE_WGS * TRACE_N) n = (size_t)TRACE_WGS * TRACE_N;
  if (hipMemcpyFromSymbol(host, HIP_SYMBOL(g_st_trace), n * 8) != hipSuccess) return -1;
  unsigned long long* z = (unsigned long long*)calloc(n, 8);
  (void)hipMemcpyToSymbol(HIP_SYMBOL(g_st_trace), z, n * 8);
  free(z);
  return 0;
}
#endif

namespace eyoc {

size_t local_rulebook_bytes(int n_out) { return (size_t)cdiv(n_out, TILE) * LR_BYTES; }

int build_local_rulebook(const int32_t* nbr_dev, int K, int n_out, unsigned char* out_dev, int* overflow_dev, hipStream_t st, int group) {
  if (n_out <= 0) return EYOC_OK;
  hipLaunchKernelGGL((k_local_rulebook<false, 4>), dim3(cdiv(n_out, TILE)), dim3(256), 0, st, nbr_dev, K, n_out, out_dev, overflow_dev, group, DeriveSrc());
  EYOC_CHECK_HIP(hipGetLastError());
  return EYOC_OK;
}

int build_local_rulebook_derived(const DeriveSrc& src, int n_out, unsigned char* out_dev, int* overflow_dev, hipStream_t st, int group) {
  if (n_out <= 0) return EYOC_OK;
  EYOC_REQUIRE(src.coords && src.parent && src.children && src.s1c && src.nc > 0, EYOC_ERR_INVALID, "build_local_rulebook_derived: incomplete octree");
  hipLaunchKernelGGL((k_local_rulebook<true, 4>), dim3(cdiv(n_out, TILE)), dim3(256), 0, st, (const int32_t*)nullptr, 27, n_out, out_dev, overflow_dev, group, src);
  EYOC_CHECK_HIP(hipGetLastError());
  return EYOC_OK;
}

#ifdef EYOC_ST_ABLATIONS
constexpr int ST_VARIANTS = 28;
#else
constexpr int ST_VARIANTS = 7;
#endif
int st_variants() { return ST_VARIANTS; }

bool spconv_st_can_fuse_tail(const SpconvArgs& a) {
  if (a.math != 1 || !a.local || a.l2norm || a.K != 27 || a.cout != 64 || a.cin % 32 != 0 || !a.out_split || a.out_perm) return false;
  const eyoc_ctx::Knobs& kn = knobs_of(a.ctx);
  const int v = kn.st_variant;
  if (!(v == 1 || v == 4 || v == 5 || v == 6)) return false;
  const int n_tiles = cdiv(a.n_out, TILE);
  return !((long long)n_tiles * (a.cout / 64) < kn.st_split_below);
}

__global__ __launch_bounds__(256) void k_tail_poison(unsigned int* __restrict__ range, float* __restrict__ out, int n, int ld, int c) {
  const unsigned int stored = __builtin_nontemporal_load(range + 4), inter = __builtin_nontemporal_load(range + 5);
  if (blockIdx.x == 0 && threadIdx.x == 0 && (stored | inter)) atomicOr(range, 1u);
  if (stored == 0u) return;
  const float qnan = __builtin_nanf("");
  for (long long i = (long long)blockIdx.x * 256 + threadIdx.x; i < (long long)n * c; i += (long long)gridDim.x * 256)
    out[(i / c) * ld + i % c] = qnan;
}

int launch_spconv_st(const SpconvArgs& a_in, const unsigned char* local_dev, hipStream_t st) {
  const SpconvArgs& a = a_in;
  EYOC_REQUIRE(a.math == 1 && local_dev && !a.l2norm && a.K == 27 && !a.perm, EYOC_ERR_INVALID, "spconv_st: unsupported layer");
  const int n_tiles = cdiv(a.n_out, TILE);
  const eyoc_ctx::Knobs& kn = knobs_of(a.ctx);
  const int split_below = kn.st_split_below;
  const int variant0 = kn.st_variant;
  const bool small = variant0 != 0 && a.cout >= 64 && a.cout <= 256 && (long long)n_tiles * (a.cout / 64) < split_below;
  const int ctg = a.cout >= 64 && !small ? 64 : 32;
  const bool wide = spconv_cc(a.cin, a.cout) == 64;
  const int n_cg = a.cout / ctg;
  EYOC_REQUIRE(a.cout % ctg == 0 && n_cg >= 1 && n_cg <= 8 && 8 % n_cg == 0 && a.cin % 32 == 0, EYOC_ERR_INVALID,
               "spconv_st: %d -> %d channels", a.cin, a.cout);
  SpconvArgs a_loc = a_in;
  a_loc.cg_local = (kn.st_cg_local && n_cg > 1 && variant0 != 0 && (size_t)27 * a.cin * a.cout * 4 <= (size_t)2 << 20) ? 1 : 0;
  const SpconvArgs& a2 = a_loc;
  dim3 grid((unsigned)(a_loc.cg_local ? cdiv(n_tiles, 8) * 8 * n_cg : cdiv(n_tiles, 8 / n_cg) * 8)), block(NW * 64);
  const int variant = kn.st_variant;
  int ksplit = 1;
  if (variant == 1 && ctg == 32 && a.ks_part && kn.st_ksplit && a.cin >= 128) {
    const int wgs = (int)grid.x, nqb = a.cin / 32;
    ksplit = KS_MAX_SLOTS / (wgs > 0 ? wgs : 1);
    if (ksplit > nqb) ksplit = nqb;
    if (ksplit < 4 || (long long)n_tiles * n_cg > KS_MAX_SLOTS) ksplit = 1;
    grid.y = (unsigned)ksplit;
  }
  if (variant == 0) {
#define EYOC_ST(NTW_, CC_, NH_)                                                                                             \
  do {                                                                                                                      \
    EYOC_CHECK_HIP(hipFuncSetAttribute(reinterpret_cast<const void*>(spconv_st_kernel<NTW_, CC_, NH_>),                     \
                                       hipFuncAttributeMaxDynamicSharedMemorySize, X_BYTES));                               \
    hipLaunchKernelGGL((spconv_st_kernel<NTW_, CC_, NH_>), grid, block, (size_t)X_BYTES, st, a, local_dev, n_tiles);        \
  } while (0)
    if (ctg == 64) { if (wide) EYOC_ST(2, 64, 2); else EYOC_ST(2, 32, 2); }
    else { if (wide) EYOC_ST(2, 64, 1); else EYOC_ST(2, 32, 1); }
#undef EYOC_ST
  } else {
#define EYOC_STA(CC_, NH_, SK_)                                                                                          \
  do {                                                                                                                  \
    hipLaunchKernelGGL((spconv_st_asm_kernel<CC_, NH_, SK_>), grid, block, 0, st, a2, local_dev, n_tiles, ksplit, 0);    \
    if (ksplit > 1)                                                                                                     \
      hipLaunchKernelGGL((spconv_st_asm_kernel<CC_, NH_, SK_>), dim3(grid.x), block, 0, st, a2, local_dev, n_tiles, ksplit, 1); \
  } while (0)
    if (ctg == 64) {
      if (variant == 2) { if (wide) EYOC_STA(64, 2, 0); else EYOC_STA(32, 2, 0); }
#ifdef EYOC_ST_ABLATIONS
      else if (variant == 3) { if (wide) EYOC_STA(64, 2, 2); else EYOC_STA(32, 2, 2); }
      else if (variant == 13) EYOC_STA(64, 2, 3);
      else if (variant == 14) EYOC_STA(64, 2, 4);
      else if (variant == 15) EYOC_STA(64, 2, 5);
      else if (variant == 16) EYOC_STA(64, 2, 6);
      else if (variant == 17) EYOC_STA(64, 2, 7);
      else if (variant == 18) EYOC_STA(64, 2, 8);
      else if (variant == 19) EYOC_STA(64, 2, 9);
      else if (variant == 20) EYOC_STA(64, 2, 10);
      else if (variant == 21) EYOC_STA(64, 2, 11);
      else if (variant == 22) EYOC_STA(64, 2, 12);
      else if (variant == 23) EYOC_STA(64, 2, 13);
      else if (variant == 24) EYOC_STA(64, 2, 14);
      else if (variant == 25) EYOC_STA(64, 2, 15);
      else if (variant == 26) EYOC_STA(64, 2, 16);
      else if (variant == 27) EYOC_STA(64, 2, 17);
#endif
      else if (a.tail.out) {
        EYOC_REQUIRE(spconv_st_can_fuse_tail(a) && a.range, EYOC_ERR_INVALID, "spconv_st: this layer cannot carry the fused tail");
        if (wide) hipLaunchKernelGGL((spconv_st_asm_kernel<64, 2, 1, NW, TILE, 1>), grid, block, 0, st, a2, local_dev, n_tiles, 1, 0);
        else hipLaunchKernelGGL((spconv_st_asm_kernel<32, 2, 1, NW, TILE, 1>), grid, block, 0, st, a2, local_dev, n_tiles, 1, 0);
        hipLaunchKernelGGL(k_tail_poison, dim3(256), dim3(256), 0, st, a.range, a.tail.out, a.n_out, a.tail.ld_out, 32);
      }
      else { if (wide) EYOC_STA(64, 2, 1); else EYOC_STA(32, 2, 1); }
    } else if (variant == 4) { if (wide) EYOC_STA(64, 1, 1); else EYOC_STA(32, 1, 1); }
    else if (variant == 5) { if (wide) EYOC_STA(64, 1, 19); else EYOC_STA(32, 1, 19); }
    else if (variant == 6) { if (wide) EYOC_STA(64, 1, 20); else EYOC_STA(32, 1, 20); }
    else { if (wide) EYOC_STA(64, 1, 18); else EYOC_STA(32, 1, 18); }
#undef EYOC_STA
  }
  EYOC_CHECK_HIP(hipGetLastError());
  return EYOC_OK;
}

int launch_spconv_st128(const SpconvArgs& a, const unsigned char* local_dev, hipStream_t st) {
  EYOC_REQUIRE(a.math == 1 && local_dev && !a.l2norm && a.K == 27 && !a.perm, EYOC_ERR_INVALID, "spconv_st128: unsupported layer");
  const eyoc_ctx::Knobs& kn128 = knobs_of(a.ctx);
  const bool wide_wg = a.cout % 128 == 0 && kn128.st128_wide != 0;
  const int n_tiles = cdiv(a.n_out, 128), n_cg = a.cout / (wide_wg ? 128 : 64);
  EYOC_REQUIRE(a.cout % 64 == 0 && n_cg >= 1 && n_cg <= 8 && 8 % n_cg == 0 && a.cin % 32 == 0, EYOC_ERR_INVALID, "spconv_st128: %d -> %d channels",
               a.cin, a.cout);
  const dim3 grid((unsigned)(cdiv(n_tiles, 8 / n_cg) * 8)), block(NW * 64);
  if (wide_wg) {
    if (spconv_cc(a.cin, a.cout) == 64) hipLaunchKernelGGL((spconv_st_asm_kernel<64, 2, 1, NW, 128>), grid, block, 0, st, a, local_dev, n_tiles, 1, 0);
    else hipLaunchKernelGGL((spconv_st_asm_kernel<32, 2, 1, NW, 128>), grid, block, 0, st, a, local_dev, n_tiles, 1, 0);
    EYOC_CHECK_HIP(hipGetLastError());
    return EYOC_OK;
  }
  const int nh1 = knobs_of(a.ctx).st_variant;
  const bool deep = nh1 != 4;
#ifdef EYOC_ST_ABLATIONS
  const int v_ = knobs_of(a.ctx).st_variant;
#define EYOC_ST128_ABL(SK_)                                                                                                         \
  do {                                                                                                                              \
    if (spconv_cc(a.cin, a.cout) == 64) hipLaunchKernelGGL((spconv_st_asm_kernel<64, 1, SK_, NW, 128>), grid, block, 0, st, a, local_dev, n_tiles, 1, 0); \
    else hipLaunchKernelGGL((spconv_st_asm_kernel<32, 1, SK_, NW, 128>), grid, block, 0, st, a, local_dev, n_tiles, 1, 0);          \
    EYOC_CHECK_HIP(hipGetLastError());                                                                                              \
    return EYOC_OK;                                                                                                                 \
  } while (0)
  if (v_ == 16) EYOC_ST128_ABL(6);
  if (v_ == 17) EYOC_ST128_ABL(7);
  if (v_ == 23) EYOC_ST128_ABL(13);
  if (v_ == 18) EYOC_ST128_ABL(8);
  if (v_ == 19) EYOC_ST128_ABL(9);
  if (v_ == 20) EYOC_ST128_ABL(10);
  if (v_ == 21) EYOC_ST128_ABL(11);
#undef EYOC_ST128_ABL
#endif
  if (nh1 == 5 || nh1 == 6) {
    if (spconv_cc(a.cin, a.cout) == 64) {
// ... 31 lines not shown
```

### eyoc_amd/csrc/spconv_upc.hip

```cpp
#include <atomic>

#include "spconv.h"
#include "derive.h"

using namespace eyoc;

namespace {

typedef float f32x16 __attribute__((ext_vector_type(16)));
typedef unsigned int u32x8 __attribute__((ext_vector_type(8)));
typedef unsigned int u32x4 __attribute__((ext_vector_type(4)));

constexpr int NW = 4;
constexpr int TILE = NW * 64;
constexpr int XROWS = 640;
constexpr int UMAX = XROWS - 1;
constexpr int NPASS = 2;
constexpr int UCAP = NPASS * XROWS;
constexpr int X_BYTES = XROWS * 128;
constexpr int LO_REGION = XROWS * 64;
constexpr int KC = 8;
__host__ __device__ constexpr int slot_addr(int l) { return l * 64 + ((l >> 2) & 3) * 16; }

constexpr int U_OFF = 16;
constexpr int LOC_OFF = U_OFF + UCAP * 4;
constexpr int MASK_OFF = LOC_OFF + NPASS * KC * 64 * 8;
constexpr int OROW_OFF = MASK_OFF + NPASS * KC * 2;
constexpr int UPC_LR = (OROW_OFF + TILE * 4 + 127) / 128 * 128;
static_assert(OROW_OFF % 16 == 0 && LOC_OFF % 16 == 0, "16-byte accesses");

__host__ __device__ constexpr int class_of(int k) { return (k % 3 != 1 ? 1 : 0) | ((k / 3) % 3 != 1 ? 2 : 0) | (k / 9 != 1 ? 4 : 0); }
struct ClassTable {
  int order[27];
  int start[9];
};
constexpr ClassTable make_classes() {
  ClassTable t{};
  int n = 0;
  for (int b = 0; b < 8; ++b) {
    t.start[b] = n;
    for (int k = 0; k < 27; ++k)
      if (class_of(k) == b) t.order[n++] = k;
  }
  t.start[8] = n;
  return t;
}
__constant__ ClassTable c_classes = make_classes();
constexpr int MIN_TILE_ROWS = 128;
__device__ int g_tile_rows[8] = {256, 256, 256, 256, 256, 256, 256, 192};
__device__ inline int tile_rows(int b) { return g_tile_rows[b]; }

struct UpcHeader {
  int n_tiles;
  int tile_start[9];
  int count[8];
  int overflow;
};
constexpr int HDR_BYTES = 256;

constexpr int PBLK = 1024;
__global__ __launch_bounds__(256) void k_upc_class(const int32_t* __restrict__ nbr, const int32_t* __restrict__ coords, int stride, int n,
                                                   unsigned char* __restrict__ cls, int* __restrict__ blk_cnt) {
  __shared__ int cnt[NW][8];
  const int lane = threadIdx.x & 63, wave = threadIdx.x >> 6;
  int mine[8] = {0, 0, 0, 0, 0, 0, 0, 0};
#pragma unroll
  for (int i = 0; i < PBLK / 256; ++i) {
    const int row = blockIdx.x * PBLK + i * 256 + (int)threadIdx.x;
    int c = 8;
    if (row < n) {
      if (coords) {
        const int4 q = reinterpret_cast<const int4*>(coords)[row];
        c = ((q.y / stride) & 1) | (((q.z / stride) & 1) << 1) | (((q.w / stride) & 1) << 2);
      } else {
        c = 0;
#pragma unroll
        for (int k = 26; k >= 0; --k)
          if (nbr[(size_t)k * n + row] >= 0) c = class_of(k);
      }
      cls[row] = (unsigned char)c;
    }
#pragma unroll
    for (int b = 0; b < 8; ++b) mine[b] += __popcll(__ballot(c == b));
  }
  if (lane == 0)
#pragma unroll
    for (int b = 0; b < 8; ++b) cnt[wave][b] = mine[b];
  __syncthreads();
  if (threadIdx.x < 8) blk_cnt[blockIdx.x * 8 + threadIdx.x] = cnt[0][threadIdx.x] + cnt[1][threadIdx.x] + cnt[2][threadIdx.x] + cnt[3][threadIdx.x];
}

__global__ __launch_bounds__(1024) void k_upc_scan(int* __restrict__ blk_cnt, int nblk, UpcHeader* __restrict__ hdr) {
  __shared__ int part[1024][8];
  const int t = (int)threadIdx.x;
  const int per = (nblk + 1023) / 1024, b0 = t * per, b1 = min(nblk, b0 + per);
  int s[8] = {0, 0, 0, 0, 0, 0, 0, 0};
  for (int b = b0; b < b1; ++b) {
    const int4 lo = reinterpret_cast<const int4*>(blk_cnt)[b * 2], hi = reinterpret_cast<const int4*>(blk_cnt)[b * 2 + 1];
    s[0] += lo.x; s[1] += lo.y; s[2] += lo.z; s[3] += lo.w; s[4] += hi.x; s[5] += hi.y; s[6] += hi.z; s[7] += hi.w;
  }
#pragma unroll
  for (int c = 0; c < 8; ++c) part[t][c] = s[c];
  __syncthreads();
  for (int d = 1; d < 1024; d <<= 1) {
    int v[8];
#pragma unroll
    for (int c = 0; c < 8; ++c) v[c] = t >= d ? part[t - d][c] : 0;
    __syncthreads();
#pragma unroll
    for (int c = 0; c < 8; ++c) part[t][c] += v[c];
    __syncthreads();
  }
  int run[8];
#pragma unroll
  for (int c = 0; c < 8; ++c) run[c] = part[t][c] - s[c];
  for (int b = b0; b < b1; ++b) {
    const int4 lo = reinterpret_cast<const int4*>(blk_cnt)[b * 2], hi = reinterpret_cast<const int4*>(blk_cnt)[b * 2 + 1];
    reinterpret_cast<int4*>(blk_cnt)[b * 2] = make_int4(run[0], run[1], run[2], run[3]);
    reinterpret_cast<int4*>(blk_cnt)[b * 2 + 1] = make_int4(run[4], run[5], run[6], run[7]);
    run[0] += lo.x; run[1] += lo.y; run[2] += lo.z; run[3] += lo.w; run[4] += hi.x; run[5] += hi.y; run[6] += hi.z; run[7] += hi.w;
  }
  if (t == 0) {
    int tiles = 0;
    for (int c = 0; c < 8; ++c) {
      const int total = part[1023][c];
      hdr->count[c] = total;
      hdr->tile_start[c] = tiles;
      tiles += (total + tile_rows(c) - 1) / tile_rows(c);
    }
    hdr->tile_start[8] = tiles;
    hdr->n_tiles = tiles;
    hdr->overflow = 0;
  }
}

__global__ __launch_bounds__(256) void k_upc_scatter(const unsigned char* __restrict__ cls, int n, const int* __restrict__ blk_base,
                                                     const UpcHeader* __restrict__ hdr, int* __restrict__ sorted) {
  __shared__ int cnt[PBLK / 256][NW][8];
  const int lane = threadIdx.x & 63, wave = threadIdx.x >> 6;
  int c[PBLK / 256], rank[PBLK / 256];
#pragma unroll
  for (int i = 0; i < PBLK / 256; ++i) {
    const int row = blockIdx.x * PBLK + i * 256 + (int)threadIdx.x;
    c[i] = row < n ? (int)cls[row] : 8;
    rank[i] = 0;
#pragma unroll
    for (int b = 0; b < 8; ++b) {
      const unsigned long long m = __ballot(c[i] == b);
      if (c[i] == b) rank[i] = __popcll(m & ((1ull << lane) - 1ull));
      if (lane == 0) cnt[i][wave][b] = __popcll(m);
    }
  }
  __syncthreads();
#pragma unroll
  for (int i = 0; i < PBLK / 256; ++i) {
    if (c[i] >= 8) continue;
    int r = rank[i];
    for (int q = 0; q < i * NW + wave; ++q) r += cnt[q / NW][q % NW][c[i]];
    const int pos = blk_base[blockIdx.x * 8 + c[i]] + r, R = tile_rows(c[i]);
    sorted[(size_t)(hdr->tile_start[c[i]] + pos / R) * TILE + pos % R] = blockIdx.x * PBLK + i * 256 + (int)threadIdx.x;
  }
}

__global__ __launch_bounds__(256) void k_upc_order(const UpcHeader* __restrict__ hdr, int* __restrict__ tile_order) {
  const int t = blockIdx.x * 256 + (int)threadIdx.x;
  if (t >= hdr->n_tiles) return;
  int b = 0;
  while (t >= hdr->tile_start[b + 1]) ++b;
  const long long ti = t - hdr->tile_start[b], Tb = hdr->tile_start[b + 1] - hdr->tile_start[b];
  int rank = 0;
  for (int o = 0; o < 8; ++o) {
    const long long To = hdr->tile_start[o + 1] - hdr->tile_start[o];
    if (To == 0) continue;
    if (o == b) { rank += (int)ti; continue; }
    const long long A = (2 * ti + 1) * To;
    const long long q = o < b ? A / Tb : (A + Tb - 1) / Tb - 1;
    long long cnt = q >= 1 ? (q - 1) / 2 + 1 : 0;
    if (cnt > To) cnt = To;
    rank += (int)cnt;
  }
  tile_order[rank] = t;
}

constexpr int HSLOTS = 4096;
__global__ __launch_bounds__(256) void k_upc_records(const int32_t* __restrict__ nbr, int n, const int* __restrict__ sorted,
                                                     UpcHeader* __restrict__ hdr, unsigned char* __restrict__ out, int compact) {
  __shared__ int hk[HSLOTS];
  __shared__ unsigned short hid[HSLOTS], hpos[HSLOTS];
  __shared__ unsigned short srow[KC][TILE];
  __shared__ __attribute__((aligned(16))) unsigned int key[TILE];
  __shared__ int wave_cnt[NW];
  __shared__ unsigned char nib[NPASS][KC][NW];
  const int tile = blockIdx.x;
  if (tile >= hdr->n_tiles) return;
  const int lane = threadIdx.x & 63, wave = threadIdx.x >> 6;
  int b = 0;
  while (tile >= hdr->tile_start[b + 1]) ++b;
  const int k0 = c_classes.start[b], nk = c_classes.start[b + 1] - k0;
  const int row = sorted[(size_t)tile * TILE + threadIdx.x];
  for (int i = threadIdx.x; i < HSLOTS; i += 256) hk[i] = -1;
  __syncthreads();
  int idxs[KC];
#pragma unroll
  for (int i = 0; i < KC; ++i) {
    const int k = c_classes.order[k0 + (i < nk ? i : 0)];
    idxs[i] = (i < nk && row >= 0) ? nbr[(size_t)(compact ? up8_slot_of_offset(k) : k) * n + row] : -1;
  }
  unsigned int pattern = 0;
#pragma unroll
  for (int i = 0; i < KC; ++i) {
    const int idx = idxs[i];
    unsigned int s = 0xFFFFu;
    if (idx >= 0) {
      pattern |= 1u << i;
      s = ((unsigned)idx * 2654435761u) >> 20;
      while (true) {
        const int prev = atomicCAS(&hk[s], -1, idx);
        if (prev == -1 || prev == idx) break;
        s = (s + 1) & (HSLOTS - 1);
      }
    }
    srow[i][threadIdx.x] = (unsigned short)s;
  }
  key[threadIdx.x] = (pattern << 8) | threadIdx.x;
  __syncthreads();
  constexpr int PER_WAVE = HSLOTS / NW;
  int cnt = 0;
  for (int i0 = 0; i0 < PER_WAVE; i0 += 64) cnt += __popcll(__ballot(hk[wave * PER_WAVE + i0 + lane] >= 0));
  if (lane == 0) wave_cnt[wave] = cnt;
  __syncthreads();
  int base = 0, total = 0;
  for (int w = 0; w < NW; ++w) { if (w < wave) base += wave_cnt[w]; total += wave_cnt[w]; }
  unsigned char* lr = out + (size_t)tile * UPC_LR;
  int* U = reinterpret_cast<int*>(lr + U_OFF);
  if (total <= UMAX) {
    for (int i0 = 0; i0 < PER_WAVE; i0 += 64) {
      const int s = wave * PER_WAVE + i0 + lane;
      const int kv = hk[s];
      const unsigned long long m = __ballot(kv >= 0);
      const int id = base + __popcll(m & ((1ull << lane) - 1ull));
      if (kv >= 0) {
        hid[s] = (unsigned short)id;
        U[id] = kv;
      }
      base += __popcll(m);
    }
  } else {
    for (int i0 = 0; i0 < PER_WAVE; i0 += 64) {
      const int s = wave * PER_WAVE + i0 + lane;
      const unsigned long long m = __ballot(hk[s] >= 0);
      if (hk[s] >= 0) hpos[s] = (unsigned short)(base + __popcll(m & ((1ull << lane) - 1ull)));
      base += __popcll(m);
    }
    __syncthreads();
    for (int i0 = 0; i0 < PER_WAVE; i0 += 64) {
      const int s = wave * PER_WAVE + i0 + lane;
      const int kv = hk[s];
      if (kv >= 0) {
        const int id = canonical_slot_id<HSLOTS>(hk, hpos, s);
        hid[s] = (unsigned short)id;
        if (id < NPASS * UMAX) U[id] = kv;
      }
    }
  }
  if (threadIdx.x == 0) {
    reinterpret_cast<int*>(lr)[0] = total <= NPASS * UMAX ? total : -1;
    reinterpret_cast<int*>(lr)[1] = b;
    if (total > NPASS * UMAX) atomicAdd(&hdr->overflow, 1);
  }
  {
    const unsigned int mine = key[threadIdx.x];
    int rank = 0;
    const uint4* kp = reinterpret_cast<const uint4*>(key);
#pragma unroll 8
    for (int i = 0; i < TILE / 4; ++i) {
      const uint4 kk = kp[i];
      rank += (kk.x < mine) + (kk.y < mine) + (kk.z < mine) + (kk.w < mine);
    }
    __syncthreads();
    key[rank] = mine;
    __syncthreads();
  }
  const int r = (int)threadIdx.x, w = r >> 6, c = (r >> 4) & 3, j = r & 15;
  const int src = (int)(key[(c * 4 + ((c & 1) ? 3 - w : w)) * 16 + j] & 255u);
  const int orow = sorted[(size_t)tile * TILE + src];
  reinterpret_cast<int*>(lr + OROW_OFF)[(w * 16 + j) * 4 + c] = orow;
  unsigned short* loc = reinterpret_cast<unsigned short*>(lr + LOC_OFF);
#pragma unroll
  for (int i = 0; i < KC; ++i) {
    if (i >= nk) break;
    const unsigned int hs = srow[i][src];
    const int id = hs != 0xFFFFu ? (int)hid[hs] : -1;
#pragma unroll
    for (int p = 0; p < NPASS; ++p) {
      if (p > 0 && total <= p * UMAX) continue;
      const int l = (id >= p * UMAX && id < (p + 1) * UMAX) ? id - p * UMAX : UMAX;
      loc[(((size_t)(p * KC + i) * 64) + w * 16 + j) * 4 + c] = (unsigned short)slot_addr(l);
      const unsigned long long bl = __ballot(l != UMAX);
      if (lane == 0)
        nib[p][i][w] = (unsigned char)(((bl & 0xFFFFull) != 0) | (((bl >> 16) & 0xFFFFull) != 0) << 1 | (((bl >> 32) & 0xFFFFull) != 0) << 2 |
                                       (((bl >> 48) & 0xFFFFull) != 0) << 3);
    }
  }
  __syncthreads();
  if (threadIdx.x < NPASS * KC) {
    const int p = (int)threadIdx.x / KC, i = (int)threadIdx.x % KC;
    unsigned short m = 0;
    if (i < nk && !(p > 0 && total <= p * UMAX)) m = (unsigned short)(nib[p][i][0] | nib[p][i][1] << 4 | nib[p][i][2] << 8 | nib[p][i][3] << 12);
    reinterpret_cast<unsigned short*>(lr + MASK_OFF)[p * KC + i] = m;
  }
}

#include "spconv_st_loop.inc"
#ifdef EYOC_UPC_ABL
#include "spconv_st_loop_abl.inc"
#if EYOC_UPC_ABL == 1
#define EYOC_UPC_BLOB EYOC_ST_LOOP_UPC_NOM
#elif EYOC_UPC_ABL == 2
#define EYOC_UPC_BLOB EYOC_ST_LOOP_UPC_NOW
#elif EYOC_UPC_ABL == 3
#define EYOC_UPC_BLOB EYOC_ST_LOOP_UPC_EMPTY
#else
#define EYOC_UPC_BLOB EYOC_ST_LOOP_UPC
#endif
#else
#define EYOC_UPC_ABL 0
#define EYOC_UPC_BLOB EYOC_ST_LOOP_UPC
#endif

template <int CC>
__global__ __launch_bounds__(NW * 64, 2) void spconv_upc_kernel(SpconvArgs a, const unsigned char* __restrict__ ws, int max_tiles) {
  constexpr int NTW = 2, CTW = NTW * 16, NC = 4, NH = 2, CTG = 64;
  constexpr int NITV = XROWS / (16 * NW);
  __shared__ __attribute__((aligned(128))) unsigned char xs[X_BYTES];
  const UpcHeader* hdr = reinterpret_cast<const UpcHeader*>(ws);
  const int n_tiles = __builtin_amdgcn_readfirstlane(hdr->n_tiles);
  const int lane = threadIdx.x & 63;
  const int wave = __builtin_amdgcn_readfirstlane((int)(threadIdx.x >> 6));
  const int g = lane >> 4, j = lane & 15;
  const int n_cg = a.cout / CTG;
  const int xcd = (int)blockIdx.x & 7, seq = (int)blockIdx.x >> 3;
  const int per_xcd = (n_tiles + 7) >> 3;
  const int e = xcd * per_xcd + seq / n_cg, cg = seq % n_cg;
  if (seq / n_cg >= per_xcd || e >= n_tiles) return;
  const int* tile_order = reinterpret_cast<const int*>(ws + HDR_BYTES);
  const int tile = __builtin_amdgcn_readfirstlane(tile_order[e]);
  const unsigned char* lr = ws + HDR_BYTES + (((size_t)max_tiles * 4 + 255) & ~(size_t)255) + (size_t)tile * UPC_LR;
  const int w0 = 2 * (wave >> 1);
  const int ct0 = cg * CTG + (wave & 1) * CTW;
  const int CT = a.cout >= 128 ? 128 : a.cout;
  const int n_slices = a.cout / CT, slice = ct0 / CT, nt0 = (ct0 - slice * CT) / 16;
  constexpr int JQ = CC / 16;
  const int ncc = a.cin / CC;
  const int nqb = a.cin / 32;

  const int* __restrict__ U = reinterpret_cast<const int*>(lr + U_OFF);
  if (threadIdx.x < 8)
    *reinterpret_cast<float4*>(xs + (threadIdx.x >> 2) * LO_REGION + UMAX * 64 + (threadIdx.x & 3) * 16) = make_float4(0.f, 0.f, 0.f, 0.f);
  const unsigned long long wbits = (unsigned long long)(size_t)a.w;
  u32x4 wr;
  wr[0] = (unsigned)__builtin_amdgcn_readfirstlane((int)(unsigned)wbits);
  wr[1] = (unsigned)__builtin_amdgcn_readfirstlane((int)((unsigned)(wbits >> 32) & 0xFFFFu));
  wr[2] = (unsigned)__builtin_amdgcn_readfirstlane(27 * a.cin * a.cout * 4);
  wr[3] = 0x00020000u;
  const int tile4 = CC * CT / 4;
  const unsigned int kstride = (unsigned)(n_slices * ncc * tile4 * 16);
  const unsigned int w1off = JQ * 1024;
  if ((unsigned)(size_t)(__attribute__((address_space(3))) unsigned char*)xs != 0u) __builtin_trap();

  f32x16 A0, A1, A2, A3;
#pragma unroll
  for (int i = 0; i < 16; ++i) { A0[i] = 0.f; A1[i] = 0.f; A2[i] = 0.f; A3[i] = 0.f; }

  int n_up = 0;
  int Ureg[NITV];
  auto load_rows = [&](int pass) {
#pragma unroll
    for (int it = 0; it < NITV; ++it) Ureg[it] = U[pass * UMAX + (it * NW + wave) * 16 + (lane >> 2)];
  };
  auto stage = [&](int qb) {
    if (EYOC_UPC_ABL == 4) return;
#pragma unroll
    for (int it = 0; it < NITV; ++it) {
      const int l0 = (it * NW + wave) * 16;
      if (l0 < n_up) {
        const int l = l0 + (lane >> 2);
        const float* src = a.in + (size_t)Ureg[it] * a.ld_in + qb * 32 + (((lane & 3) ^ ((l >> 2) & 3)) << 2);
        if (l < n_up) {
          __builtin_amdgcn_global_load_lds(src, (__attribute__((address_space(3))) void*)(xs + l0 * 64), 16, 0, 0);
          __builtin_amdgcn_global_load_lds(src + 16, (__attribute__((address_space(3))) void*)(xs + LO_REGION + l0 * 64), 16, 0, 0);
        }
      }
    }
  };

  load_rows(0);
  int warm = 0;
  if (threadIdx.x < KC * 64 * 8 / 128) warm = *reinterpret_cast<const int*>(lr + LOC_OFF + threadIdx.x * 128);
  const int n_u = __builtin_amdgcn_readfirstlane(reinterpret_cast<const int*>(lr)[0]);
  const int cls = __builtin_amdgcn_readfirstlane(reinterpret_cast<const int*>(lr)[1]);
  const int k0 = c_classes.start[cls], nk = c_classes.start[cls + 1] - k0;
  u32x8 KO;
#pragma unroll
  for (int i = 0; i < 8; ++i) KO[i] = (unsigned)__builtin_amdgcn_readfirstlane(c_classes.order[k0 + (i < nk ? i : 0)]) * kstride;
  const int n_pass = n_u > UMAX ? 2 : 1;
  bool first = true;
  for (int pass = 0; pass < n_pass; ++pass) {
    n_up = min(n_u - pass * UMAX, UMAX);
    if (pass > 0) load_rows(pass);
    const unsigned int* mp = reinterpret_cast<const unsigned int*>(lr + MASK_OFF + pass * KC * 2);
    u32x8 M0;
#pragma unroll
    for (int i = 0; i < 8; ++i) M0[i] = i < 4 ? (unsigned)__builtin_amdgcn_readfirstlane((int)mp[i]) >> (w0 * 4) : 0u;
    const unsigned char* lb = lr + LOC_OFF + ((size_t)pass * KC * 64 + w0 * 16) * 8;
    for (int qb = 0; qb < nqb; ++qb) {
      if (!first) __syncthreads();
      first = false;
      stage(qb);
      const int cc = (qb * 32) / CC, qp = ((qb * 32) % CC) / 32;
      const unsigned int ws0 = (unsigned)__builtin_amdgcn_readfirstlane(((slice * ncc + cc) * tile4 + (nt0 * JQ + 2 * qp) * 64) * 16);
      unsigned int so;
      asm volatile(EYOC_UPC_BLOB : "+{v[64:79]}"(A0), "+{v[80:95]}"(A1), "+{v[96:111]}"(A2), "+{v[112:127]}"(A3), [so] "=&s"(so)
                   : [wr] "s"(wr), [ws0] "s"(ws0), [lb] "s"(lb), [w1] "s"(w1off), [nk] "s"(nk), "{s[36:43]}"(M0), "{s[52:59]}"(KO)
                   : "memory", "scc", EYOC_ST_LOOP_CLOBBERS);
    }
  }
  asm volatile("" :: "v"(warm));

  const float os = a.out_scale ? *a.out_scale : 1.0f;
  const int ch = ct0 + 8 * g;
  float4 b4[NTW];
#pragma unroll
  for (int t = 0; t < NTW; ++t)
    b4[t] = a.bias ? *reinterpret_cast<const float4*>(a.bias + ch + 4 * t) : make_float4(0.f, 0.f, 0.f, 0.f);
  float mx = 0.f;
  constexpr int NG = NH * NC;
  int orow[NG];
#pragma unroll
  for (int h = 0; h < NH; ++h) {
    const int4 rm = *reinterpret_cast<const int4*>(lr + OROW_OFF + ((w0 + h) * 16 + j) * 16);
    orow[h * NC + 0] = rm.x; orow[h * NC + 1] = rm.y; orow[h * NC + 2] = rm.z; orow[h * NC + 3] = rm.w;
  }
  float4 v[NG][NTW];
#pragma unroll
  for (int hc = 0; hc < NG; ++hc) {
    const int o = orow[hc];
#pragma unroll
    for (int t = 0; t < NTW; ++t) {
      const int ai = (hc * NTW + t) * 4;
      const f32x16& A = ai < 16 ? A0 : ai < 32 ? A1 : ai < 48 ? A2 : A3;
      v[hc][t] = make_float4(A[ai % 16 + 0] * os + b4[t].x, A[ai % 16 + 1] * os + b4[t].y, A[ai % 16 + 2] * os + b4[t].z,
                             A[ai % 16 + 3] * os + b4[t].w);
      if (a.relu) { v[hc][t].x = fmaxf(v[hc][t].x, 0.f); v[hc][t].y = fmaxf(v[hc][t].y, 0.f); v[hc][t].z = fmaxf(v[hc][t].z, 0.f); v[hc][t].w = fmaxf(v[hc][t].w, 0.f); }
      if (o >= 0) split16_track(mx, v[hc][t]);
    }
  }
#pragma unroll
  for (int hc = 0; hc < NG; ++hc) {
    const int o = orow[hc];
    if (o < 0) continue;
    if (EYOC_UPC_ABL == 5 && os != 12345.f) continue;
    if (a.out_split) {
      uint2 h0, l0, h1, l1;
      split16_encode4(v[hc][0], h0, l0);
      split16_encode4(v[hc][1], h1, l1);
      char* op = reinterpret_cast<char*>(a.out + (size_t)o * a.ld_out) + split16_off4(ch);
      *reinterpret_cast<uint4*>(op) = make_uint4(h0.x, h0.y, h1.x, h1.y);
      *reinterpret_cast<uint4*>(op + SPLIT16_LO) = make_uint4(l0.x, l0.y, l1.x, l1.y);
    } else {
      float* op = a.out + (size_t)o * a.ld_out + ch;
      *reinterpret_cast<float4*>(op) = v[hc][0];
      *reinterpret_cast<float4*>(op + 4) = v[hc][1];
    }
  }
  if (a.out_split) split16_report(a.range, mx);
}

}

namespace eyoc {

static inline int upc_max_tiles(int n_out) { return cdiv(n_out, MIN_TILE_ROWS) + 8; }
static inline size_t upc_records_off(int n_out) { return (size_t)HDR_BYTES + (((size_t)upc_max_tiles(n_out) * 4 + 255) & ~(size_t)255); }

size_t upc_kept_bytes(int n_out) { return n_out <= 0 ? 0 : upc_records_off(n_out) + (size_t)upc_max_tiles(n_out) * UPC_LR; }
size_t upc_scratch_bytes(int n_out) {
  if (n_out <= 0) return 0;
  const size_t nblk = (size_t)cdiv(n_out, PBLK);
  return (((size_t)n_out + 255) & ~(size_t)255) + nblk * 8 * 4 + 256 + (size_t)upc_max_tiles(n_out) * TILE * 4;
}

int build_upc(const int32_t* nbr_dev, const int32_t* coords_dev, int stride, int n_out, unsigned char* ws, unsigned char* scratch, hipStream_t st,
              bool compact) {
  EYOC_REQUIRE(!compact || coords_dev, EYOC_ERR_INVALID, "build_upc: the compact table needs the level's coordinates for the classes");
  if (n_out <= 0) return EYOC_OK;
  const int nblk = cdiv(n_out, PBLK), max_tiles = upc_max_tiles(n_out);
  unsigned char* cls = scratch;
  int* blk = reinterpret_cast<int*>(scratch + (((size_t)n_out + 255) & ~(size_t)255));
  int* sorted = reinterpret_cast<int*>(reinterpret_cast<unsigned char*>(blk) + (size_t)nblk * 8 * 4 + 256);
  UpcHeader* hdr = reinterpret_cast<UpcHeader*>(ws);
  int* order = reinterpret_cast<int*>(ws + HDR_BYTES);
  EYOC_CHECK_HIP(hipMemsetAsync(sorted, 0xFF, (size_t)max_tiles * TILE * 4, st));
  hipLaunchKernelGGL(k_upc_class, dim3(nblk), dim3(256), 0, st, nbr_dev, coords_dev, stride, n_out, cls, blk);
  hipLaunchKernelGGL(k_upc_scan, dim3(1), dim3(1024), 0, st, blk, nblk, hdr);
  hipLaunchKernelGGL(k_upc_scatter, dim3(nblk), dim3(256), 0, st, cls, n_out, blk, hdr, sorted);
  hipLaunchKernelGGL(k_upc_order, dim3(cdiv(max_tiles, 256)), dim3(256), 0, st, hdr, order);
  hipLaunchKernelGGL(k_upc_records, dim3(max_tiles), dim3(256), 0, st, nbr_dev, n_out, sorted, hdr, ws + upc_records_off(n_out), compact ? 1 : 0);
  EYOC_CHECK_HIP(hipGetLastError());
  return EYOC_OK;
}

int upc_set_tile_rows(int odd_axes, int rows) {
  if (odd_axes < 0 || odd_axes > 3 || rows < MIN_TILE_ROWS || rows > TILE || rows % 16) return EYOC_ERR_INVALID;
  int h[8];
  EYOC_CHECK_HIP(hipMemcpyFromSymbol(h, HIP_SYMBOL(g_tile_rows), sizeof(h)));
  for (int b = 0; b < 8; ++b)
    if (__builtin_popcount(b) == odd_axes) h[b] = rows;
  EYOC_CHECK_HIP(hipMemcpyToSymbol(HIP_SYMBOL(g_tile_rows), h, sizeof(h)));
  return EYOC_OK;
}

const int* upc_overflow_ptr(const unsigned char* ws) { return &reinterpret_cast<const UpcHeader*>(ws)->overflow; }

int launch_spconv_upc(const SpconvArgs& a, const unsigned char* ws, hipStream_t st) {
  EYOC_REQUIRE(a.math == 1 && ws && !a.l2norm && a.K == 27 && !a.res && !a.out_perm, EYOC_ERR_INVALID, "spconv_upc: unsupported layer");
  EYOC_REQUIRE(a.cout % 64 == 0 && a.cout <= 512 && a.cin % 32 == 0, EYOC_ERR_INVALID, "spconv_upc: %d -> %d channels", a.cin, a.cout);
  if (a.n_out <= 0) return EYOC_OK;
  const int max_tiles = upc_max_tiles(a.n_out), n_cg = a.cout / 64;
  const dim3 grid((unsigned)(cdiv(max_tiles, 8) * n_cg * 8)), block(NW * 64);
  if (spconv_cc(a.cin, a.cout) == 64) hipLaunchKernelGGL((spconv_upc_kernel<64>), grid, block, 0, st, a, ws, max_tiles);
  else hipLaunchKernelGGL((spconv_upc_kernel<32>), grid, block, 0, st, a, ws, max_tiles);
  EYOC_CHECK_HIP(hipGetLastError());
  return EYOC_OK;
}

}
```

### include/eyoc_hip.h

```cpp
#ifndef EYOC_HIP_H
#define EYOC_HIP_H

#include <stddef.h>
#include <stdint.h>

#ifdef __cplusplus
extern "C" {
#endif

typedef struct eyoc_ctx eyoc_ctx;
typedef struct eyoc_maps eyoc_maps;
typedef struct eyoc_model eyoc_model;

typedef enum {
  EYOC_OK = 0,
  EYOC_ERR_INVALID = -1,
  EYOC_ERR_HIP = -2,
  EYOC_ERR_WORKSPACE = -3,
  EYOC_ERR_DUPLICATE = -4,
  EYOC_ERR_RANGE = -5
} eyoc_status;

#define EYOC_MAX_LEVELS 4
#define EYOC_VERSION 111

int eyoc_version(void);
const char* eyoc_last_error(void);
int eyoc_create(int device, eyoc_ctx** out);
int eyoc_destroy(eyoc_ctx* ctx);

typedef enum { EYOC_MAP_S1 = 0, EYOC_MAP_DOWN = 1, EYOC_MAP_UP = 2 } eyoc_map_kind;

typedef struct {
  int32_t n_levels;
  int32_t rows[EYOC_MAX_LEVELS];
  int64_t pairs_s1[EYOC_MAX_LEVELS];
  int64_t pairs_down[EYOC_MAX_LEVELS];
  int64_t pairs_up[EYOC_MAX_LEVELS];
  int64_t pairs_conv1;
} eyoc_maps_info_t;

size_t eyoc_maps_workspace_bytes(int n_rows);
int eyoc_maps_build(eyoc_ctx* ctx, const int32_t* coords_dev, int n_rows, void* workspace_dev,
                    size_t workspace_bytes, void* stream, eyoc_maps** out);
int eyoc_maps_build_ordered(eyoc_ctx* ctx, const int32_t* coords_dev, int n_rows, void* workspace_dev,
                            size_t workspace_bytes, void* stream, int order, eyoc_maps** out);
int eyoc_maps_last_fault_batches(const eyoc_ctx* ctx, uint32_t* dup, uint32_t* range);
int eyoc_maps_free(eyoc_maps* maps);
int eyoc_maps_copy_up_order(const eyoc_maps* maps, int level, int32_t* out_dev, void* stream);
int eyoc_maps_order_min_rows(eyoc_ctx* ctx, int min_rows);
int eyoc_maps_order_window_shift(eyoc_ctx* ctx, int shift);
int eyoc_maps_select_orders(eyoc_ctx* ctx, int s1, int down);
int eyoc_maps_internal_order(eyoc_ctx* ctx, int mode);
int eyoc_maps_lazy_tables(eyoc_ctx* ctx, int on);
int eyoc_maps_fused_levels(eyoc_ctx* ctx, int on);
int eyoc_spconv_select_down_kernel(eyoc_ctx* ctx, int mode);
const int32_t* eyoc_maps_row_order(const eyoc_maps* maps);
int eyoc_maps_copy_row_order(const eyoc_maps* maps, int32_t* out_dev, void* stream);
int eyoc_maps_rows(const eyoc_maps* maps, int level);
const int32_t* eyoc_maps_coords(const eyoc_maps* maps, int level);
const int32_t* eyoc_maps_table(const eyoc_maps* maps, int kind, int level);
int eyoc_maps_copy_coords(const eyoc_maps* maps, int level, int32_t* out_dev, void* stream);
int eyoc_maps_copy_table(const eyoc_maps* maps, int kind, int level, int32_t* out_dev, void* stream);
int eyoc_maps_info(eyoc_ctx* ctx, const eyoc_maps* maps, int conv1_kernel_size, void* stream,
                   eyoc_maps_info_t* info);

size_t eyoc_voxelize_workspace_bytes(int n_points);
int eyoc_voxelize(eyoc_ctx* ctx, const float* xyz_dev, int n_points, int stride, float voxel_size, int batch_index,
                  int32_t* sel_dev, int32_t* coords_dev, int* n_out, void* workspace_dev, size_t workspace_bytes,
                  void* stream);

size_t eyoc_voxelize_batched_workspace_bytes(int n_points_total, int n_clouds);
int eyoc_voxelize_batched(eyoc_ctx* ctx, const float* xyz_dev, int stride, const int64_t* point_offsets, int n_clouds,
                          int n_points, float voxel_size, int batch_base, int32_t* sel_dev, int32_t* coords_dev,
                          float* xyz_out_dev, int64_t* voxel_offsets, void* workspace_dev, size_t workspace_bytes,
                          void* stream);
size_t eyoc_voxelize_batched_isolating_workspace_bytes(int n_points_total, int n_clouds);
int eyoc_voxelize_batched_isolating(eyoc_ctx* ctx, const float* xyz_dev, int stride, const int64_t* point_offsets, int n_clouds,
                                    int n_points, float voxel_size, int batch_base, int32_t* sel_dev, int32_t* coords_dev,
                                    float* xyz_out_dev, int64_t* voxel_offsets, void* workspace_dev, size_t workspace_bytes,
                                    void* stream, int32_t* cloud_faults);

size_t eyoc_batch_drop_workspace_bytes(int n_rows);
int eyoc_batch_drop(eyoc_ctx* ctx, const int32_t* coords_dev, const float* feats_dev, int n_rows, int c, const uint32_t* drop_mask,
                    int32_t* coords_out_dev, float* feats_out_dev, int32_t* row_map_dev, int* n_kept, int32_t* kept_per_batch,
                    void* workspace_dev, size_t workspace_bytes, void* stream);
int eyoc_remap_rows(eyoc_ctx* ctx, const int64_t* idx_dev, int m, const int32_t* row_map_dev, int n_rows, int64_t* out_dev,
                    void* stream);

size_t eyoc_spconv_packed_floats(int K, int cin, int cout);
int eyoc_spconv_pack_weights(const float* w_host , const float* scale_host ,
                             int K, int cin, int cout, float* packed_host);
int eyoc_spconv(eyoc_ctx* ctx, const int32_t* nbr_dev, int K, int n_out, const float* in_dev,
                int ld_in, int cin, const float* wpacked_dev, int cout, const float* bias_dev,
                const float* res_dev, int ld_res, int relu, float* out_dev, int ld_out, void* stream);
int eyoc_spconv_select_split16_kernel(eyoc_ctx* ctx, int mode);
int eyoc_spconv_select_up_kernel(eyoc_ctx* ctx, int on);
int eyoc_spconv_upc_min_rows(eyoc_ctx* ctx, int rows);
int eyoc_spconv_upc_tile_rows(int odd_axes, int rows);
size_t eyoc_spconv_upc_bytes(int n_out);
int eyoc_spconv_upc_build(eyoc_ctx* ctx, const int32_t* nbr_dev, int n_out, void* ws_dev, int32_t* info_host, void* stream);
int eyoc_spconv_upc(eyoc_ctx* ctx, const int32_t* nbr_dev, const void* ws_dev, int n_out, int n_in, const float* in_dev, int ld_in,
                    int cin, const float* wpacked_dev, int cout, const float* bias_dev, int relu, float* out_dev, int ld_out,
                    int out_split, const float* out_scale_dev, void* stream);
int eyoc_spconv_select_conv1_kernel(eyoc_ctx* ctx, int on);
int eyoc_spconv_select_st_kernel(eyoc_ctx* ctx, int variant);
int eyoc_spconv_st_split_below(eyoc_ctx* ctx, int workgroups);
int eyoc_spconv_st_group_rows(eyoc_ctx* ctx, int on);
int eyoc_spconv_st_ksplit(eyoc_ctx* ctx, int on);
size_t eyoc_spconv_local_rulebook_bytes(int n_out);
int eyoc_spconv_build_local_rulebook(eyoc_ctx* ctx, const int32_t* nbr_dev, int K, int n_out, void* out_dev,
                                     int32_t* overflow_dev, void* stream);
int eyoc_spconv_staged(eyoc_ctx* ctx, const int32_t* nbr_dev, const void* local_dev, int n_out, int n_in, const float* in_dev,
                       int ld_in, int cin, const float* wpacked_dev, int cout, const float* bias_dev, const float* res_dev,
                       int ld_res, int relu, float* out_dev, int ld_out, int out_split, const float* out_scale_dev, void* stream);
int eyoc_spconv_pack_weights_split16(const float* w_host, const float* scale_host, int K, int cin, int cout,
                                     float* packed_host, float* out_scale_host);
int eyoc_spconv_ex(eyoc_ctx* ctx, const int32_t* nbr_dev, int K, int n_out, int n_in, const float* in_dev, int ld_in, int cin,
                   const float* wpacked_dev, int cout, const float* bias_dev, const float* res_dev, int ld_res, int relu,
                   float* out_dev, int ld_out, int math, int out_split, const float* out_scale_dev, void* stream);
int eyoc_split16_encode(eyoc_ctx* ctx, const float* in_dev, int n, int c, int ld_in, float* out_dev, int ld_out, void* stream);
int eyoc_split16_decode(eyoc_ctx* ctx, const float* in_dev, int n, int c, int ld_in, float* out_dev, int ld_out, void* stream);
int eyoc_spconv_sum(eyoc_ctx* ctx, const int32_t* nbr_dev, int K, int n_out, const float* in_dev, int ld_in, int cin,
                    const float* wpacked_dev, int cout, float* out_dev, int ld_out, void* stream);
int eyoc_spconv_pack_weights_transposed(const float* w_host , int K, int cin, int cout, int mirror,
                                        float* packed_host);
size_t eyoc_spconv_grad_weight_workspace_bytes(int K, int n_out, int cin, int cout);
int eyoc_spconv_grad_weight(eyoc_ctx* ctx, const int32_t* nbr_dev, int K, int n_out, const float* in_dev, int ld_in, int cin,
                            const float* dout_dev, int ld_dout, int cout, float* dw_dev, void* workspace_dev,
                            size_t workspace_bytes, void* stream);
int eyoc_spconv_select_kernel(eyoc_ctx* ctx, int mode);

typedef struct {
  int32_t in_channels, out_channels, conv1_kernel_size, normalize_feature;
  int32_t channels[5];
  int32_t tr_channels[5];
  float bn_eps;
  int32_t expanded;
} eyoc_model_desc;

typedef struct {
  const char* name;
  const float* kernel;
  int32_t K, cin, cout;
  const float* bias;
  const float* bn_weight;
  const float* bn_bias;
  const float* bn_mean;
  const float* bn_var;
} eyoc_layer_params;

size_t eyoc_model_blob_floats(const eyoc_model_desc* desc);
int eyoc_model_pack_host(const eyoc_model_desc* desc, const eyoc_layer_params* layers, int n_layers,
                         float* blob_host, size_t blob_floats);
int eyoc_model_create(eyoc_ctx* ctx, const eyoc_model_desc* desc, const eyoc_layer_params* layers,
                      int n_layers, float* blob_dev, size_t blob_floats, eyoc_model** out);
int eyoc_model_destroy(eyoc_model* model);
int eyoc_model_fuse_tail(eyoc_ctx* ctx, int on);
size_t eyoc_model_workspace_bytes(const eyoc_model* model, const eyoc_maps* maps);
int eyoc_model_forward(eyoc_ctx* ctx, const eyoc_model* model, const eyoc_maps* maps,
                       const float* feats_dev, float* out_dev, void* workspace_dev,
                       size_t workspace_bytes, void* stream);
int eyoc_model_num_layers(const eyoc_model* model);
int eyoc_model_layer_work(eyoc_ctx* ctx, const eyoc_model* model, const eyoc_maps* maps, void* stream,
                          const char** names, int64_t* pairs, double* flops, double* gather_bytes,
                          double* compulsory_bytes);
int eyoc_model_set_math(eyoc_model* model, int mode);
int eyoc_model_last_math(const eyoc_model* model);
int eyoc_model_range_check(eyoc_model* model, void* stream, float* max_abs);
int eyoc_model_range_snapshot(eyoc_model* model, uint32_t* words_host, void* stream);
int eyoc_model_set_progress_event(eyoc_model* model, int layer, void* hip_event);
int eyoc_model_set_probe(eyoc_model* model, int on);
int eyoc_model_set_timing(eyoc_model* model, int on);
int eyoc_model_layer_ms(eyoc_model* model, float* ms );
int eyoc_model_timing_slot(eyoc_model* model, int slot);

int eyoc_knn_prefilter(eyoc_ctx* ctx, int mode);
int eyoc_knn1(eyoc_ctx* ctx, const float* A_dev, const float* B_dev, int c, const int32_t* seg_a,
              const int32_t* seg_b, int nseg, int dist_type, int64_t* idx_dev, float* dist_dev,
              void* stream);

int eyoc_gather_rows(eyoc_ctx* ctx, const float* F_dev, int ld, int c, const int64_t* sel_dev, int n,
                     const float* G_dev, float beta, float* out_dev, void* stream);

int eyoc_dotmax(eyoc_ctx* ctx, const float* A_dev, const float* B_dev, int c, const int32_t* seg_a,
                const int32_t* seg_b, int nseg, int64_t* idx_dev, float* weight_dev, void* stream);

int eyoc_knn2(eyoc_ctx* ctx, const float* A_dev, const float* B_dev, int c, const int32_t* seg_a,
              const int32_t* seg_b, int nseg, int64_t* idx_dev, float* d1_dev, float* d2_dev, void* stream);

int eyoc_lowe_topk(eyoc_ctx* ctx, const float* d1_dev, const float* d2_dev, int n, int k, int64_t* idx_out_dev,
                   float* w_out_dev, void* stream);
int eyoc_pair_filter(eyoc_ctx* ctx, int mode, const float* P0_dev, const float* P1_dev, const int64_t* idx0_dev,
                     const int64_t* idx1_dev, int m, const float* T_dev, float radius, int64_t* pairs_out_dev,
                     int32_t* n_out_dev, void* stream);

int eyoc_pair_filter_similarity(eyoc_ctx* ctx, const float* P0_dev, const float* P1_dev, const int64_t* idx0_dev,
                                const int64_t* idx1_dev, int m, const double* table_dev, int xlim, int ylim, float grid0,
                                float grid1, double thresh, int64_t* pairs_out_dev, int32_t* n_out_dev, void* stream);

int eyoc_pdist(eyoc_ctx* ctx, const float* A_dev, int n, const float* B_dev, int m, int c, int dist_type,
               float* out_dev, void* stream);

int eyoc_kabsch_batched(eyoc_ctx* ctx, const float* A_dev, const float* B_dev, const float* w_dev,
                        int bs, int n, float* T_dev, void* stream);
int eyoc_irls_quad(eyoc_ctx* ctx, const float* p0_dev, const float* p1_dev, const float* w_dev, int n,
                   int iters, float* T_dev, void* stream);

// ... 64 lines not shown
```

Before: 3367 pairs/s.

## Batch per-level rulebook and up-class builders into multi-job kernel launches

Adds a batched builder path, on by default for large clouds, that builds the local rulebooks for all pyramid levels with one grid-partitioned launch per kernel family. Each workgroup finds its job from a prefix table. The up-class partition pipeline (class, scan, scatter, order, records) is likewise launched once per stage across all levels, with a single memset over row lists laid out back to back. This cuts the number of kernel launches and lets small levels share the GPU rather than running as serial small grids, at the cost of a new workspace layout and extra job-lookup logic. It also adds ablation macros (off by default) and introspection APIs for records and job mapping.

```diff
diff --git a/eyoc_amd/_lib.py b/eyoc_amd/_lib.py
--- a/eyoc_amd/_lib.py
+++ b/eyoc_amd/_lib.py
@@ -60,6 +60,9 @@
     "eyoc_maps_internal_order": (_i, [_vp, _i]),
     "eyoc_maps_lazy_tables": (_i, [_vp, _i]),
     "eyoc_maps_fused_levels": (_i, [_vp, _i]),
+    "eyoc_maps_batched_builders": (_i, [_vp, _i]),
+    "eyoc_maps_records": (_vp, [_vp, _i, _i, C.POINTER(_sz)]),
+    "eyoc_maps_builder_job": (_i, [C.POINTER(_i), _i, _i, C.POINTER(_i), C.POINTER(_i)]),
     "eyoc_spconv_select_down_kernel": (_i, [_vp, _i]),
     "eyoc_maps_order_window_shift": (_i, [_vp, _i]),
     "eyoc_maps_row_order": (_vp, [_vp]),
diff --git a/eyoc_amd/csrc/common.h b/eyoc_amd/csrc/common.h
--- a/eyoc_amd/csrc/common.h
+++ b/eyoc_amd/csrc/common.h
@@ -78,6 +78,7 @@
     int maps_s1_order = 1, maps_down_order = 0;
     int maps_internal_order = -1;
     int maps_lazy_tables = 1, maps_fused_levels = 1;
+    int maps_batched_builders = 1;
     int knn_prefilter = 1;
     int fuse_tail = 2;
     int spconv_kernel = -1;
diff --git a/eyoc_amd/csrc/coordmap.hip b/eyoc_amd/csrc/coordmap.hip
--- a/eyoc_amd/csrc/coordmap.hip
+++ b/eyoc_amd/csrc/coordmap.hip
@@ -940,7 +940,85 @@
     }
   }
   if (zorder) {
-    for (int l = 0; l < EYOC_MAX_LEVELS; ++l) {
+    const bool use_down = kn.down_kernel == 1 && n >= kn.upc_min_rows;
+    const bool batched = kn.maps_batched_builders != 0 && n >= kn.upc_min_rows;
+    if (batched) {
+      for (int l = 0; l < EYOC_MAX_LEVELS; ++l) {
+        m->local_s1[l] = cv.take<unsigned char>(local_rulebook_bytes(m->rows[l]));
+        if (l + 1 < EYOC_MAX_LEVELS && use_up) m->local_up[l] = cv.take<unsigned char>(local_rulebook_up_bytes(m->rows[l]));
+        if (l + 1 < EYOC_MAX_LEVELS && use_upc) m->local_upc[l] = cv.take<unsigned char>(upc_kept_bytes(m->rows[l]));
+      }
+      unsigned char *scr_lo = nullptr, *scr_hi = nullptr;
+      for (int l = 0; l + 1 < EYOC_MAX_LEVELS && use_upc; ++l) {
+        unsigned char* sc = cv.take<unsigned char>(upc_scratch_bytes(m->rows[l]));
+        if (!sc) continue;
+        if (!scr_lo) scr_lo = sc;
+        scr_hi = sc + upc_scratch_bytes(m->rows[l]);
+      }
+      if (use_down && kn.s1_wide) m->local_s1w[EYOC_MAX_LEVELS - 1] = cv.take<unsigned char>(local_rulebook128_bytes(m->rows[EYOC_MAX_LEVELS - 1]));
+      for (int l = 0; l + 1 < EYOC_MAX_LEVELS && use_down; ++l) m->local_down[l] = cv.take<unsigned char>(local_rulebook128_bytes(m->rows[l + 1]));
+      if (!cv.ok()) {
+        set_error("eyoc_maps_build: internal workspace accounting error (%zu > %zu)", cv.off, cv.cap);
+        delete m;
+        return EYOC_ERR_WORKSPACE;
+      }
+      LrJob s1j[BUILD_JOBS];
+      int n_s1 = 0;
+      static_assert(EYOC_MAX_LEVELS <= BUILD_JOBS, "one job per level");
+      for (int l = 0; l < EYOC_MAX_LEVELS; ++l) {
+        if (lazy && l == 0) {
+          DeriveSrc src;
+          src.coords = m->coords[0]; src.parent = m->parent[0]; src.children = m->children[0]; src.s1c = m->nbr_s1[1];
+          src.nc = m->rows[1]; src.sh = 0; src.up8 = m->up8[0];
+          if (int rc = build_local_rulebook_derived(src, m->rows[0], m->local_s1[0], counters + 8, st, kn.st_group)) { delete m; return rc; }
+          continue;
+        }
+        LrJob& j = s1j[n_s1++];
+        j.nbr = m->nbr_s1[l]; j.out = m->local_s1[l]; j.overflow = counters + 8; j.n_out = m->rows[l];
+      }
+      if (int rc = build_local_rulebook_jobs(s1j, n_s1, false, st, kn.st_group)) { delete m; return rc; }
+      if (use_upc) {
+        UpcJob uj[BUILD_JOBS];
+        int n_up = 0;
+        unsigned char* part = scr_lo;
+        size_t sorted_total = 0;
+        for (int l = 0; l + 1 < EYOC_MAX_LEVELS; ++l)
+          if (m->local_upc[l]) sorted_total += upc_sorted_bytes(m->rows[l]);
+        unsigned char* sorted = scr_hi - sorted_total;
+        for (int l = 0; l + 1 < EYOC_MAX_LEVELS; ++l) {
+          if (!m->local_upc[l]) {
+            if (int rc = maps_ensure_table(m, EYOC_MAP_UP, l, st)) { delete m; return rc; }
+            continue;
+          }
+          UpcJob& j = uj[n_up++];
+          j.nbr = lazy ? m->up8[l] : m->nbr_up[l]; j.coords = m->coords[l]; j.stride = 1 << l; j.n_out = m->rows[l];
+          j.ws = m->local_upc[l]; j.part = part; j.sorted = sorted;
+          part += upc_part_bytes(m->rows[l]);
+          sorted += upc_sorted_bytes(m->rows[l]);
+        }
+        if (part > scr_hi - sorted_total) {
+          set_error("eyoc_maps_build: internal error - the class partition's scratch does not hold its %d levels", n_up);
+          delete m;
+          return EYOC_ERR_WORKSPACE;
+        }
+        if (int rc = build_upc_jobs(uj, n_up, st, lazy)) { delete m; return rc; }
+      }
+      for (int l = 0; l + 1 < EYOC_MAX_LEVELS && use_up; ++l)
+        if (int rc = build_local_rulebook_up(m->nbr_up[l], 27, m->rows[l], m->local_up[l], counters + 9, st)) { delete m; return rc; }
+      LrJob dj[BUILD_JOBS];
+      int n_dn = 0;
+      for (int l = 0; l + 1 < EYOC_MAX_LEVELS; ++l)
+        if (m->local_down[l]) {
+          LrJob& j = dj[n_dn++];
+          j.nbr = m->nbr_down[l]; j.out = m->local_down[l]; j.overflow = counters + 10 + l; j.n_out = m->rows[l + 1];
+        }
+      if (m->local_s1w[EYOC_MAX_LEVELS - 1]) {
+        LrJob& j = dj[n_dn++];
+        j.nbr = m->nbr_s1[EYOC_MAX_LEVELS - 1]; j.out = m->local_s1w[EYOC_MAX_LEVELS - 1]; j.overflow = counters + 13; j.n_out = m->rows[EYOC_MAX_LEVELS - 1];
+      }
+      if (int rc = build_local_rulebook_jobs(dj, n_dn, true, st, kn.st_group)) { delete m; return rc; }
+    }
+    for (int l = 0; l < EYOC_MAX_LEVELS && !batched; ++l) {
       m->local_s1[l] = cv.take<unsigned char>(local_rulebook_bytes(m->rows[l]));
       if (lazy && l == 0) {
         DeriveSrc src;
@@ -960,13 +1038,12 @@
         } else if (int rc = maps_ensure_table(m, EYOC_MAP_UP, l, st)) { delete m; return rc; }
       }
     }
-    const bool use_down = kn.down_kernel == 1 && n >= kn.upc_min_rows;
-    for (int l = EYOC_MAX_LEVELS - 1; l < EYOC_MAX_LEVELS && use_down && kn.s1_wide; ++l) {
+    for (int l = EYOC_MAX_LEVELS - 1; l < EYOC_MAX_LEVELS && use_down && kn.s1_wide && !batched; ++l) {
       m->local_s1w[l] = cv.take<unsigned char>(local_rulebook128_bytes(m->rows[l]));
       if (m->local_s1w[l])
         if (int rc = build_local_rulebook128(m->nbr_s1[l], 27, m->rows[l], m->local_s1w[l], counters + 13, st, kn.st_group)) { delete m; return rc; }
     }
-    for (int l = 0; l + 1 < EYOC_MAX_LEVELS && use_down; ++l) {
+    for (int l = 0; l + 1 < EYOC_MAX_LEVELS && use_down && !batched; ++l) {
       m->local_down[l] = cv.take<unsigned char>(local_rulebook128_bytes(m->rows[l + 1]));
       if (m->local_down[l])
         if (int rc = build_local_rulebook128(m->nbr_down[l], 27, m->rows[l + 1], m->local_down[l], counters + 10 + l, st, kn.st_group)) { delete m; return rc; }
@@ -1321,6 +1398,43 @@
   return prev;
 }
 
+int eyoc_maps_batched_builders(eyoc_ctx* ctx, int on) {
+  EYOC_REQUIRE(ctx, EYOC_ERR_INVALID, "eyoc_maps_batched_builders: NULL ctx");
+  const int prev = ctx->knobs.maps_batched_builders;
+  if (on == 0 || on == 1) ctx->knobs.maps_batched_builders = on;
+  return prev;
+}
+
+const void* eyoc_maps_records(const eyoc_maps* maps, int kind, int level, size_t* bytes) {
+  if (bytes) *bytes = 0;
+  if (!maps || level < 0 || level >= EYOC_MAX_LEVELS) return nullptr;
+  const unsigned char* p = nullptr;
+  size_t b = 0;
+  switch (kind) {
+    case 0: p = maps->local_s1[level]; b = local_rulebook_bytes(maps->rows[level]); break;
+    case 1: p = maps->local_s1w[level]; b = local_rulebook128_bytes(maps->rows[level]); break;
+    case 2: p = maps->local_down[level]; b = level + 1 < EYOC_MAX_LEVELS ? local_rulebook128_bytes(maps->rows[level + 1]) : 0; break;
+    case 3: p = maps->local_upc[level]; b = upc_kept_bytes(maps->rows[level]); break;
+    case 4: p = maps->local_up[level]; b = local_rulebook_up_bytes(maps->rows[level]); break;
+    case 5: p = reinterpret_cast<const unsigned char*>(maps->up8[level]); b = (size_t)8 * maps->rows[level] * sizeof(int32_t); break;
+    default: return nullptr;
+  }
+  if (!p || b == 0) return nullptr;
+  if (bytes) *bytes = b;
+  return p;
+}
+
+int eyoc_maps_builder_job(const int* wgs, int n_jobs, int wg, int* job, int* index) {
+  EYOC_REQUIRE(wgs && job && index && n_jobs >= 0 && n_jobs <= BUILD_JOBS, EYOC_ERR_INVALID, "eyoc_maps_builder_job: bad arguments");
+  for (int j = 0; j < n_jobs; ++j) EYOC_REQUIRE(wgs[j] >= 0, EYOC_ERR_INVALID, "eyoc_maps_builder_job: job %d has %d workgroups", j, wgs[j]);
+  int first[BUILD_JOBS + 1];
+  const int total = build_job_grid(wgs, n_jobs, first);
+  EYOC_REQUIRE(wg >= 0 && wg < total, EYOC_ERR_INVALID, "eyoc_maps_builder_job: workgroup %d outside the grid of %d", wg, total);
+  *job = build_job_of(first, wg);
+  *index = wg - first[*job];
+  return EYOC_OK;
+}
+
 int eyoc_maps_fused_levels(eyoc_ctx* ctx, int on) {
   EYOC_REQUIRE(ctx, EYOC_ERR_INVALID, "eyoc_maps_fused_levels: NULL ctx");
   const int prev = ctx->knobs.maps_fused_levels;
diff --git a/eyoc_amd/csrc/spconv.h b/eyoc_amd/csrc/spconv.h
--- a/eyoc_amd/csrc/spconv.h
+++ b/eyoc_amd/csrc/spconv.h
@@ -140,6 +140,43 @@
 int build_local_rulebook128(const int32_t* nbr_dev, int K, int n_out, unsigned char* out_dev, int* overflow_dev, hipStream_t st, int group = 1);
 int launch_spconv_st128(const SpconvArgs& a, const unsigned char* local_dev, hipStream_t st);
 int build_local_rulebook_derived(const DeriveSrc& src, int n_out, unsigned char* out_dev, int* overflow_dev, hipStream_t st, int group = 1);
+constexpr int BUILD_JOBS = 4;
+__host__ __device__ inline int build_job_of(const int* first, int wg) {
+  int j = 0;
+#pragma unroll
+  for (int i = 1; i < BUILD_JOBS; ++i) j += wg >= first[i] ? 1 : 0;
+  return j;
+}
+inline int build_job_grid(const int* wgs, int n_jobs, int* first) {
+  int total = 0;
+  for (int j = 0; j <= BUILD_JOBS; ++j) {
+    first[j] = total;
+    if (j < n_jobs) total += wgs[j];
+  }
+  return total;
+}
+struct LrJob {
+  const int32_t* nbr = nullptr;
+  unsigned char* out = nullptr;
+  int* overflow = nullptr;
+  int n_out = 0;
+};
+struct LrJobs {
+  int first[BUILD_JOBS + 1];
+  LrJob job[BUILD_JOBS];
+};
+int build_local_rulebook_jobs(const LrJob* jobs, int n_jobs, bool rows128, hipStream_t st, int group = 1);
+struct UpcJob {
+  const int32_t* nbr = nullptr;
+  const int32_t* coords = nullptr;
+  int stride = 1, n_out = 0;
+  unsigned char* ws = nullptr;
+  unsigned char* part = nullptr;
+  unsigned char* sorted = nullptr;
+};
+size_t upc_part_bytes(int n_out);
+size_t upc_sorted_bytes(int n_out);
+int build_upc_jobs(const UpcJob* jobs, int n_jobs, hipStream_t st, bool compact = false);
 int launch_spconv_rs(const SpconvArgs& a, hipStream_t st);
 bool tail_fusable(int cin1, int cmid, int cout);
 int launch_tail_fused(const float* in, int ld_in, int n, const float* w1, const float* s1, const float* b1, int relu1, const float* w2,
diff --git a/eyoc_amd/csrc/spconv_st.hip b/eyoc_amd/csrc/spconv_st.hip
--- a/eyoc_amd/csrc/spconv_st.hip
+++ b/eyoc_amd/csrc/spconv_st.hip
@@ -34,10 +34,13 @@
 #define EYOC_LR_HSLOTS_LOG2 11
 #endif
 constexpr int HSLOTS_LOG2 = EYOC_LR_HSLOTS_LOG2, HSLOTS_T = 1 << HSLOTS_LOG2;
+#ifndef EYOC_LR_ABL
+#define EYOC_LR_ABL 0
+#endif
 
 template <bool DERIVE, int NWB>
-__global__ __launch_bounds__(NWB * 64) void k_local_rulebook(const int32_t* __restrict__ nbr, int K, int n_out, unsigned char* __restrict__ out,
-                                                             int* __restrict__ overflow, int group, DeriveSrc d) {
+__device__ __forceinline__ void local_rulebook_tile(const int32_t* __restrict__ nbr, int K, int n_out, unsigned char* __restrict__ out,
+                                                    int* __restrict__ overflow, int group, const DeriveSrc& d, const int tile) {
   constexpr int TR = NWB * 64;
   constexpr int HS = HSLOTS_T, HSHIFT = 32 - HSLOTS_LOG2;
   __shared__ int hk[HS];
@@ -47,7 +50,6 @@
   __shared__ int wave_cnt[NWB];
   __shared__ int too_many;
   const int lane = threadIdx.x & 63, wave = threadIdx.x >> 6;
-  const int tile = blockIdx.x;
   const int row = tile * TR + (int)threadIdx.x;
   for (int i = threadIdx.x; i < HS; i += TR) hk[i] = -1;
   if (threadIdx.x == 0) too_many = 0;
@@ -82,7 +84,8 @@
     if (idx >= 0) {
       s = ((unsigned)idx * 2654435761u) >> HSHIFT;
       int probes = 0;
-      while (true) {
+      if (EYOC_LR_ABL == 2) hk[s] = idx;
+      else while (true) {
         const int prev = atomicCAS(&hk[s], -1, idx);
         if (prev == -1 || prev == idx) break;
         s = (s + 1) & (HS - 1);
@@ -173,10 +176,11 @@
     int rank = 0;
     const ulonglong2* kp = reinterpret_cast<const ulonglong2*>(key);
 #pragma unroll 8
-    for (int i = 0; i < TR / 2; ++i) {
+    for (int i = 0; i < (EYOC_LR_ABL == 1 ? 0 : TR / 2); ++i) {
       const ulonglong2 kk = kp[i];
       rank += (kk.x < mine) + (kk.y < mine);
     }
+    if (EYOC_LR_ABL == 1) rank = (int)threadIdx.x;
     __syncthreads();
     key[rank] = mine;
     __syncthreads();
@@ -189,7 +193,7 @@
   lr[RM_OFF + (w * 16 + j) * 4 + c] = (unsigned char)src;
   lr[INV_OFF + src] = (unsigned char)r;
 #pragma unroll
-  for (int k = 0; k < 27; ++k) {
+  for (int k = 0; k < (EYOC_LR_ABL == 3 ? 0 : 27); ++k) {
     const unsigned int hs = srow[k][src];
     const int id = hs != 0xFFFFu ? (int)hid[hs] : -1;
 #pragma unroll
@@ -213,6 +217,19 @@
     }
     reinterpret_cast<unsigned short*>(msk)[p * 28 + k] = m;
   }
+}
+
+template <bool DERIVE, int NWB>
+__global__ __launch_bounds__(NWB * 64) void k_local_rulebook(const int32_t* __restrict__ nbr, int K, int n_out, unsigned char* __restrict__ out,
+                                                             int* __restrict__ overflow, int group, DeriveSrc d) {
+  local_rulebook_tile<DERIVE, NWB>(nbr, K, n_out, out, overflow, group, d, (int)blockIdx.x);
+}
+
+template <int NWB>
+__global__ __launch_bounds__(NWB * 64) void k_local_rulebook_jobs(LrJobs a, int group) {
+  const int j = __builtin_amdgcn_readfirstlane(build_job_of(a.first, (int)blockIdx.x));
+  const LrJob jb = a.job[j];
+  local_rulebook_tile<false, NWB>(jb.nbr, 27, jb.n_out, jb.out, jb.overflow, group, DeriveSrc(), (int)blockIdx.x - a.first[j]);
 }
 
 template <int NTW, int CC, int NH>
@@ -876,6 +893,22 @@
 int build_local_rulebook(const int32_t* nbr_dev, int K, int n_out, unsigned char* out_dev, int* overflow_dev, hipStream_t st, int group) {
   if (n_out <= 0) return EYOC_OK;
   hipLaunchKernelGGL((k_local_rulebook<false, 4>), dim3(cdiv(n_out, TILE)), dim3(256), 0, st, nbr_dev, K, n_out, out_dev, overflow_dev, group, DeriveSrc());
+  EYOC_CHECK_HIP(hipGetLastError());
+  return EYOC_OK;
+}
+
+int build_local_rulebook_jobs(const LrJob* jobs, int n_jobs, bool rows128, hipStream_t st, int group) {
+  EYOC_REQUIRE(n_jobs >= 0 && n_jobs <= BUILD_JOBS, EYOC_ERR_INVALID, "build_local_rulebook_jobs: %d jobs", n_jobs);
+  LrJobs a;
+  int wgs[BUILD_JOBS];
+  for (int j = 0; j < n_jobs; ++j) {
+    a.job[j] = jobs[j];
+    wgs[j] = jobs[j].n_out > 0 ? cdiv(jobs[j].n_out, rows128 ? 128 : TILE) : 0;
+  }
+  const int total = build_job_grid(wgs, n_jobs, a.first);
+  if (total <= 0) return EYOC_OK;
+  if (rows128) hipLaunchKernelGGL((k_local_rulebook_jobs<2>), dim3(total), dim3(128), 0, st, a, group);
+  else hipLaunchKernelGGL((k_local_rulebook_jobs<4>), dim3(total), dim3(256), 0, st, a, group);
   EYOC_CHECK_HIP(hipGetLastError());
   return EYOC_OK;
 }
diff --git a/eyoc_amd/csrc/spconv_upc.hip b/eyoc_amd/csrc/spconv_upc.hip
--- a/eyoc_amd/csrc/spconv_upc.hip
+++ b/eyoc_amd/csrc/spconv_upc.hip
@@ -59,14 +59,14 @@
 constexpr int HDR_BYTES = 256;
 
 constexpr int PBLK = 1024;
-__global__ __launch_bounds__(256) void k_upc_class(const int32_t* __restrict__ nbr, const int32_t* __restrict__ coords, int stride, int n,
-                                                   unsigned char* __restrict__ cls, int* __restrict__ blk_cnt) {
+__device__ __forceinline__ void upc_class_block(const int32_t* __restrict__ nbr, const int32_t* __restrict__ coords, int stride, int n,
+                                                unsigned char* __restrict__ cls, int* __restrict__ blk_cnt, const int block) {
   __shared__ int cnt[NW][8];
   const int lane = threadIdx.x & 63, wave = threadIdx.x >> 6;
   int mine[8] = {0, 0, 0, 0, 0, 0, 0, 0};
 #pragma unroll
   for (int i = 0; i < PBLK / 256; ++i) {
-    const int row = blockIdx.x * PBLK + i * 256 + (int)threadIdx.x;
+    const int row = block * PBLK + i * 256 + (int)threadIdx.x;
     int c = 8;
     if (row < n) {
       if (coords) {
@@ -87,10 +87,14 @@
 #pragma unroll
     for (int b = 0; b < 8; ++b) cnt[wave][b] = mine[b];
   __syncthreads();
-  if (threadIdx.x < 8) blk_cnt[blockIdx.x * 8 + threadIdx.x] = cnt[0][threadIdx.x] + cnt[1][threadIdx.x] + cnt[2][threadIdx.x] + cnt[3][threadIdx.x];
-}
-
-__global__ __launch_bounds__(1024) void k_upc_scan(int* __restrict__ blk_cnt, int nblk, UpcHeader* __restrict__ hdr) {
+  if (threadIdx.x < 8) blk_cnt[block * 8 + threadIdx.x] = cnt[0][threadIdx.x] + cnt[1][threadIdx.x] + cnt[2][threadIdx.x] + cnt[3][threadIdx.x];
+}
+__global__ __launch_bounds__(256) void k_upc_class(const int32_t* __restrict__ nbr, const int32_t* __restrict__ coords, int stride, int n,
+                                                   unsigned char* __restrict__ cls, int* __restrict__ blk_cnt) {
+  upc_class_block(nbr, coords, stride, n, cls, blk_cnt, (int)blockIdx.x);
+}
+
+__device__ __forceinline__ void upc_scan_block(int* __restrict__ blk_cnt, int nblk, UpcHeader* __restrict__ hdr) {
   __shared__ int part[1024][8];
   const int t = (int)threadIdx.x;
   const int per = (nblk + 1023) / 1024, b0 = t * per, b1 = min(nblk, b0 + per);
@@ -133,15 +137,18 @@
     hdr->overflow = 0;
   }
 }
-
-__global__ __launch_bounds__(256) void k_upc_scatter(const unsigned char* __restrict__ cls, int n, const int* __restrict__ blk_base,
-                                                     const UpcHeader* __restrict__ hdr, int* __restrict__ sorted) {
+__global__ __launch_bounds__(1024) void k_upc_scan(int* __restrict__ blk_cnt, int nblk, UpcHeader* __restrict__ hdr) {
+  upc_scan_block(blk_cnt, nblk, hdr);
+}
+
+__device__ __forceinline__ void upc_scatter_block(const unsigned char* __restrict__ cls, int n, const int* __restrict__ blk_base,
+                                                  const UpcHeader* __restrict__ hdr, int* __restrict__ sorted, const int block) {
   __shared__ int cnt[PBLK / 256][NW][8];
   const int lane = threadIdx.x & 63, wave = threadIdx.x >> 6;
   int c[PBLK / 256], rank[PBLK / 256];
 #pragma unroll
   for (int i = 0; i < PBLK / 256; ++i) {
-    const int row = blockIdx.x * PBLK + i * 256 + (int)threadIdx.x;
+    const int row = block * PBLK + i * 256 + (int)threadIdx.x;
     c[i] = row < n ? (int)cls[row] : 8;
     rank[i] = 0;
 #pragma unroll
@@ -157,13 +164,17 @@
     if (c[i] >= 8) continue;
     int r = rank[i];
     for (int q = 0; q < i * NW + wave; ++q) r += cnt[q / NW][q % NW][c[i]];
-    const int pos = blk_base[blockIdx.x * 8 + c[i]] + r, R = tile_rows(c[i]);
-    sorted[(size_t)(hdr->tile_start[c[i]] + pos / R) * TILE + pos % R] = blockIdx.x * PBLK + i * 256 + (int)threadIdx.x;
-  }
-}
-
-__global__ __launch_bounds__(256) void k_upc_order(const UpcHeader* __restrict__ hdr, int* __restrict__ tile_order) {
-  const int t = blockIdx.x * 256 + (int)threadIdx.x;
+    const int pos = blk_base[block * 8 + c[i]] + r, R = tile_rows(c[i]);
+    sorted[(size_t)(hdr->tile_start[c[i]] + pos / R) * TILE + pos % R] = block * PBLK + i * 256 + (int)threadIdx.x;
+  }
+}
+__global__ __launch_bounds__(256) void k_upc_scatter(const unsigned char* __restrict__ cls, int n, const int* __restrict__ blk_base,
+                                                     const UpcHeader* __restrict__ hdr, int* __restrict__ sorted) {
+  upc_scatter_block(cls, n, blk_base, hdr, sorted, (int)blockIdx.x);
+}
+
+__device__ __forceinline__ void upc_order_block(const UpcHeader* __restrict__ hdr, int* __restrict__ tile_order, const int block) {
+  const int t = block * 256 + (int)threadIdx.x;
   if (t >= hdr->n_tiles) return;
   int b = 0;
   while (t >= hdr->tile_start[b + 1]) ++b;
@@ -181,17 +192,19 @@
   }
   tile_order[rank] = t;
 }
+__global__ __launch_bounds__(256) void k_upc_order(const UpcHeader* __restrict__ hdr, int* __restrict__ tile_order) {
+  upc_order_block(hdr, tile_order, (int)blockIdx.x);
+}
 
 constexpr int HSLOTS = 4096;
-__global__ __launch_bounds__(256) void k_upc_records(const int32_t* __restrict__ nbr, int n, const int* __restrict__ sorted,
-                                                     UpcHeader* __restrict__ hdr, unsigned char* __restrict__ out, int compact) {
+__device__ __forceinline__ void upc_records_tile(const int32_t* __restrict__ nbr, int n, const int* __restrict__ sorted,
+                                                 UpcHeader* __restrict__ hdr, unsigned char* __restrict__ out, int compact, const int tile) {
   __shared__ int hk[HSLOTS];
   __shared__ unsigned short hid[HSLOTS], hpos[HSLOTS];
   __shared__ unsigned short srow[KC][TILE];
   __shared__ __attribute__((aligned(16))) unsigned int key[TILE];
   __shared__ int wave_cnt[NW];
   __shared__ unsigned char nib[NPASS][KC][NW];
-  const int tile = blockIdx.x;
   if (tile >= hdr->n_tiles) return;
   const int lane = threadIdx.x & 63, wave = threadIdx.x >> 6;
   int b = 0;
@@ -309,6 +322,50 @@
     if (i < nk && !(p > 0 && total <= p * UMAX)) m = (unsigned short)(nib[p][i][0] | nib[p][i][1] << 4 | nib[p][i][2] << 8 | nib[p][i][3] << 12);
     reinterpret_cast<unsigned short*>(lr + MASK_OFF)[p * KC + i] = m;
   }
+}
+__global__ __launch_bounds__(256) void k_upc_records(const int32_t* __restrict__ nbr, int n, const int* __restrict__ sorted,
+                                                     UpcHeader* __restrict__ hdr, unsigned char* __restrict__ out, int compact) {
+  upc_records_tile(nbr, n, sorted, hdr, out, compact, (int)blockIdx.x);
+}
+
+struct UpcDevJob {
+  const int32_t* nbr;
+  const int32_t* coords;
+  unsigned char* cls;
+  int* blk;
+  int* sorted;
+  UpcHeader* hdr;
+  int* order;
+  unsigned char* records;
+  int stride, n, nblk;
+};
+struct UpcDevJobs {
+  int first_blk[BUILD_JOBS + 1], first_ord[BUILD_JOBS + 1], first_tile[BUILD_JOBS + 1];
+  UpcDevJob job[BUILD_JOBS];
+};
+__global__ __launch_bounds__(256) void k_upc_class_jobs(UpcDevJobs a) {
+  const int j = __builtin_amdgcn_readfirstlane(build_job_of(a.first_blk, (int)blockIdx.x));
+  const UpcDevJob& jb = a.job[j];
+  upc_class_block(jb.nbr, jb.coords, jb.stride, jb.n, jb.cls, jb.blk, (int)blockIdx.x - a.first_blk[j]);
+}
+__global__ __launch_bounds__(1024) void k_upc_scan_jobs(UpcDevJobs a) {
+  const UpcDevJob& jb = a.job[blockIdx.x];
+  upc_scan_block(jb.blk, jb.nblk, jb.hdr);
+}
+__global__ __launch_bounds__(256) void k_upc_scatter_jobs(UpcDevJobs a) {
+  const int j = __builtin_amdgcn_readfirstlane(build_job_of(a.first_blk, (int)blockIdx.x));
+  const UpcDevJob& jb = a.job[j];
+  upc_scatter_block(jb.cls, jb.n, jb.blk, jb.hdr, jb.sorted, (int)blockIdx.x - a.first_blk[j]);
+}
+__global__ __launch_bounds__(256) void k_upc_order_jobs(UpcDevJobs a) {
+  const int j = __builtin_amdgcn_readfirstlane(build_job_of(a.first_ord, (int)blockIdx.x));
+  const UpcDevJob& jb = a.job[j];
+  upc_order_block(jb.hdr, jb.order, (int)blockIdx.x - a.first_ord[j]);
+}
+__global__ __launch_bounds__(256) void k_upc_records_jobs(UpcDevJobs a, int compact) {
+  const int j = __builtin_amdgcn_readfirstlane(build_job_of(a.first_tile, (int)blockIdx.x));
+  const UpcDevJob& jb = a.job[j];
+  upc_records_tile(jb.nbr, jb.n, jb.sorted, jb.hdr, jb.records, compact, (int)blockIdx.x - a.first_tile[j]);
 }
 
 #include "spconv_st_loop.inc"
@@ -484,11 +541,13 @@
 static inline size_t upc_records_off(int n_out) { return (size_t)HDR_BYTES + (((size_t)upc_max_tiles(n_out) * 4 + 255) & ~(size_t)255); }
 
 size_t upc_kept_bytes(int n_out) { return n_out <= 0 ? 0 : upc_records_off(n_out) + (size_t)upc_max_tiles(n_out) * UPC_LR; }
-size_t upc_scratch_bytes(int n_out) {
+size_t upc_part_bytes(int n_out) {
   if (n_out <= 0) return 0;
   const size_t nblk = (size_t)cdiv(n_out, PBLK);
-  return (((size_t)n_out + 255) & ~(size_t)255) + nblk * 8 * 4 + 256 + (size_t)upc_max_tiles(n_out) * TILE * 4;
-}
+  return (((size_t)n_out + 255) & ~(size_t)255) + nblk * 8 * 4 + 256;
+}
+size_t upc_sorted_bytes(int n_out) { return n_out <= 0 ? 0 : (size_t)upc_max_tiles(n_out) * TILE * 4; }
+size_t upc_scratch_bytes(int n_out) { return upc_part_bytes(n_out) + upc_sorted_bytes(n_out); }
 
 int build_upc(const int32_t* nbr_dev, const int32_t* coords_dev, int stride, int n_out, unsigned char* ws, unsigned char* scratch, hipStream_t st,
               bool compact) {
@@ -510,6 +569,44 @@
   return EYOC_OK;
 }
 
+int build_upc_jobs(const UpcJob* jobs, int n_jobs, hipStream_t st, bool compact) {
+  EYOC_REQUIRE(n_jobs >= 0 && n_jobs <= BUILD_JOBS, EYOC_ERR_INVALID, "build_upc_jobs: %d jobs", n_jobs);
+  UpcDevJobs a;
+  int blks[BUILD_JOBS], ords[BUILD_JOBS], tiles[BUILD_JOBS], n_live = 0;
+  unsigned char *fill_lo = nullptr, *fill_hi = nullptr;
+  for (int j = 0; j < n_jobs; ++j) {
+    const UpcJob& u = jobs[j];
+    EYOC_REQUIRE(!compact || u.coords, EYOC_ERR_INVALID, "build_upc_jobs: the compact table needs the level's coordinates for the classes");
+    if (u.n_out <= 0) continue;
+    const int nblk = cdiv(u.n_out, PBLK), max_tiles = upc_max_tiles(u.n_out);
+    UpcDevJob& d = a.job[n_live];
+    d.nbr = u.nbr; d.coords = u.coords; d.stride = u.stride; d.n = u.n_out; d.nblk = nblk;
+    d.cls = u.part;
+    d.blk = reinterpret_cast<int*>(u.part + (((size_t)u.n_out + 255) & ~(size_t)255));
+    d.sorted = reinterpret_cast<int*>(u.sorted);
+    d.hdr = reinterpret_cast<UpcHeader*>(u.ws);
+    d.order = reinterpret_cast<int*>(u.ws + HDR_BYTES);
+    d.records = u.ws + upc_records_off(u.n_out);
+    EYOC_REQUIRE(!fill_hi || u.sorted == fill_hi, EYOC_ERR_INVALID, "build_upc_jobs: the jobs' row lists must be carved back to back");
+    if (!fill_lo) fill_lo = u.sorted;
+    fill_hi = u.sorted + upc_sorted_bytes(u.n_out);
+    blks[n_live] = nblk; ords[n_live] = cdiv(max_tiles, 256); tiles[n_live] = max_tiles;
+    ++n_live;
+  }
+  if (n_live == 0) return EYOC_OK;
+  for (int j = n_live; j < BUILD_JOBS; ++j) a.job[j] = a.job[0];
+  const int g_blk = build_job_grid(blks, n_live, a.first_blk), g_ord = build_job_grid(ords, n_live, a.first_ord),
+            g_tile = build_job_grid(tiles, n_live, a.first_tile);
+  EYOC_CHECK_HIP(hipMemsetAsync(fill_lo, 0xFF, (size_t)(fill_hi - fill_lo), st));
+  hipLaunchKernelGGL(k_upc_class_jobs, dim3(g_blk), dim3(256), 0, st, a);
+  hipLaunchKernelGGL(k_upc_scan_jobs, dim3(n_live), dim3(1024), 0, st, a);
+  hipLaunchKernelGGL(k_upc_scatter_jobs, dim3(g_blk), dim3(256), 0, st, a);
+  hipLaunchKernelGGL(k_upc_order_jobs, dim3(g_ord), dim3(256), 0, st, a);
+  hipLaunchKernelGGL(k_upc_records_jobs, dim3(g_tile), dim3(256), 0, st, a, compact ? 1 : 0);
+  EYOC_CHECK_HIP(hipGetLastError());
+  return EYOC_OK;
+}
+
 int upc_set_tile_rows(int odd_axes, int rows) {
   if (odd_axes < 0 || odd_axes > 3 || rows < MIN_TILE_ROWS || rows > TILE || rows % 16) return EYOC_ERR_INVALID;
   int h[8];
diff --git a/include/eyoc_hip.h b/include/eyoc_hip.h
--- a/include/eyoc_hip.h
+++ b/include/eyoc_hip.h
@@ -54,6 +54,9 @@
 int eyoc_maps_internal_order(eyoc_ctx* ctx, int mode);
 int eyoc_maps_lazy_tables(eyoc_ctx* ctx, int on);
 int eyoc_maps_fused_levels(eyoc_ctx* ctx, int on);
+int eyoc_maps_batched_builders(eyoc_ctx* ctx, int on);
+const void* eyoc_maps_records(const eyoc_maps* maps, int kind, int level, size_t* bytes);
+int eyoc_maps_builder_job(const int* wgs, int n_jobs, int wg, int* job, int* index);
 int eyoc_spconv_select_down_kernel(eyoc_ctx* ctx, int mode);
 const int32_t* eyoc_maps_row_order(const eyoc_maps* maps);
 int eyoc_maps_copy_row_order(const eyoc_maps* maps, int32_t* out_dev, void* stream);
```

Result: no change. 3374 pairs/s, median of 4 (+0.2%).
